# JCBrouwer/maua-style

Hardware: AMD Instinct MI355X
Metric: optimizer iterations/sec at 1024x1024 VGG-19 (higher is better)
Workload: dtype f32 (fp16x3 split-precision MFMA, fp32 accumulate)

## Files before the change

include/maua_hip.h:

```cpp
#ifndef MAUA_HIP_H
#define MAUA_HIP_H

#include <stddef.h>
#include <stdint.h>

#ifdef __cplusplus
extern "C" {
#endif

typedef void* maua_stream_t;

#define MAUA_OK 0
#define MAUA_E_INVAL (-1)
#define MAUA_E_UNSUPPORTED (-2)
#define MAUA_E_WORKSPACE (-3)

int maua_abi_version(void);
const char* maua_last_error(void);


int maua_conv_pack_filters(const float* w_oihw, float* wf, float* wb, int cout, int cin, int kh, int kw,
                           maua_stream_t stream);

size_t maua_conv_workspace_bytes(int n, int cin, int h, int w, int cout, int kh, int kw, int stride, int pad);
// ... 136 lines not shown
                                    const float* grad_scale, float* dmat, double* ledger, int slot, void* workspace, size_t workspace_bytes,
                                    maua_stream_t stream);
int maua_guided_gram_bwd_masked(const float* d_sym, const float* f, const float* guides, const float* coef, const float* mean,
                                const float* relu_mask, float* gf, int regions, int c, int64_t hw, int accumulate, maua_stream_t stream);

int maua_gram_shift_supported(int shifts, int c, int h, int w);
size_t maua_gram_shift_workspace_bytes(int shifts, int c, int h, int w);
int maua_gram_shift_fwd(const float* f, const float* mean, const int* axes, const int* deltas, const double* scales, float* gram, int shifts,
                        int c, int h, int w, void* workspace, size_t workspace_bytes, maua_stream_t stream);
int maua_gram_shift_bwd(const float* d, const float* f, const float* mean, const int* axes, const int* deltas, const double* coefs, float* gx,
                        int shifts, int c, int h, int w, int accumulate, maua_stream_t stream);

int maua_gram_flip_supported(int mirrors, int c, int h, int w);
size_t maua_gram_flip_workspace_bytes(int mirrors, int c, int h, int w);
int maua_gram_flip_fwd(const float* f, const float* mean, const int* kinds, const double* scales, float* gram, int mirrors, int c, int h, int w,
                       void* workspace, size_t workspace_bytes, maua_stream_t stream);
int maua_gram_flip_bwd(const float* d, const float* f, const float* mean, const int* kinds, const double* coefs, float* gx, int mirrors, int c,
                       int h, int w, int accumulate, maua_stream_t stream);

int maua_feat_hist_supported(int c, int h, int w, int bins, int knots);
size_t maua_feat_hist_workspace_bytes(int c, int h, int w, int bins, int knots);
size_t maua_feat_hist_state_bytes(int c, int bins);
int maua_feat_hist_fwd(const float* f, const float* table, void* state, float* loss, int c, int h, int w, int bins, int knots, void* workspace,
                       size_t workspace_bytes, maua_stream_t stream);
int maua_feat_hist_bwd(const float* f, const float* table, const void* state, const float* upstream, double coef, float* gx, int c, int h, int w,
                       int bins, int knots, int accumulate, maua_stream_t stream);

int maua_mrf_supported(int c, int h, int w, int hs, int ws, int p);
size_t maua_mrf_workspace_bytes(int c, int h, int w, int hs, int ws, int p);
size_t maua_mrf_state_bytes(int h, int w);
int maua_mrf_bank(const float* s, const int* origin, float* inv, int c, int hs, int ws, int p, maua_stream_t stream);
int maua_mrf_fwd(const float* f, const float* s, const int* origin, const float* inv, void* state, float* loss, int c, int h, int w, int hs, int ws,
                 int p, void* workspace, size_t workspace_bytes, maua_stream_t stream);
int maua_mrf_bwd(const float* f, const float* s, const int* origin, const void* state, const float* upstream, double coef, float* gx, int c, int h,
                 int w, int hs, int ws, int p, int accumulate, maua_stream_t stream);

int maua_swd_supported(int c, int d, int h, int w, int bins, int knots);
size_t maua_swd_workspace_bytes(int c, int d, int h, int w, int bins, int knots);
size_t maua_swd_state_bytes(int d, int bins);
int maua_swd_project(const float* f, const float* dirs, float* proj, void* state, int c, int d, int h, int w, int bins, void* workspace,
                     size_t workspace_bytes, maua_stream_t stream);
int maua_swd_match(float* proj_inout, const float* table, void* state, float* loss, int d, int h, int w, int bins, int knots, void* workspace,
                   size_t workspace_bytes, maua_stream_t stream);
int maua_swd_bwd(const float* g, const float* dirs_t, const float* upstream, double coef, float* gx, int c, int d, int h, int w, int accumulate,
                 maua_stream_t stream);

int maua_shift_gram_mse_ledger_supported(int shifts, int c);
int maua_shift_gram_fwd_mse_ledger(const float* f, const float* mean, const int* axes, const int* deltas, const double* scales, float* gram,
                                   int shifts, int c, int h, int w, const float* target, const double* loss_scales, const double* grad_scales,
                                   float* dmat, double* ledger, int slot, void* workspace, size_t workspace_bytes, maua_stream_t stream);
int maua_shift_gram_bwd_masked(const float* d, const float* f, const float* mean, const int* axes, const int* deltas, const double* coefs,
                               const float* relu_mask, float* gx, int shifts, int c, int h, int w, int accumulate, maua_stream_t stream);
int maua_flip_gram_mse_ledger_supported(int mirrors, int c);
int maua_flip_gram_fwd_mse_ledger(const float* f, const float* mean, const int* kinds, const double* scales, float* gram, int mirrors, int c,
                                  int h, int w, const float* target, const double* loss_scales, const double* grad_scales, float* dmat,
                                  double* ledger, int slot, void* workspace, size_t workspace_bytes, maua_stream_t stream);
int maua_flip_gram_bwd_masked(const float* d, const float* f, const float* mean, const int* kinds, const double* coefs, const float* relu_mask,
                              float* gx, int mirrors, int c, int h, int w, int accumulate, maua_stream_t stream);

int maua_tv_fwd_bwd(const float* x, float* grad, int n, int c, int h, int w, float strength, int accumulate,
                    float* loss_out, void* workspace, size_t workspace_bytes, maua_stream_t stream);

size_t maua_loss_ledger_bytes(int frames, int slots);
int maua_mse_fwd_bwd_ledger(const float* x, const float* target, float* grad, int64_t count, float loss_scale, float grad_scale,
                            int accumulate, int mask_grad_by_x, double* ledger, int slot, maua_stream_t stream);
int maua_tv_fwd_bwd_ledger(const float* x, float* grad, int n, int c, int h, int w, float strength, int accumulate,
                           double* ledger, int slot, maua_stream_t stream);
int maua_gram_mse_ledger_supported(int c);
int maua_gram_fwd_mse_ledger(const float* f, float* gram, float* row_mean_out, int c, int64_t hw, float scale, int center,
                             const float* target, float* dmat, float loss_scale, float grad_scale, double* ledger, int slot,
                             void* workspace, size_t workspace_bytes, maua_stream_t stream);
int maua_gram_partial(const float* f, float* row_mean_out, int c, int64_t hw, int center, void* workspace, size_t workspace_bytes,
                      maua_stream_t stream);
int maua_gram_partial_batch(int count, const float* const* fs, float* const* means, const int* cs, const int64_t* hws,
                            void* const* workspaces, const size_t* workspace_bytes, const int* slab_counts, maua_stream_t stream);
int maua_gram_row_means(const float* f, float* row_mean_out, int c, int64_t hw, void* workspace, size_t workspace_bytes, maua_stream_t stream);
int maua_gram_finish_mse_batch(int count, const void* const* workspaces, float* const* grams, const float* const* targets,
                               float* const* dmats, const int* cs, const int64_t* hws, const float* scales, const float* loss_scales,
                               const float* grad_scales, double* const* ledgers, const int* slots, const int* slab_counts,
                               maua_stream_t stream);
int maua_loss_ledger_sum(double* ledger, int frames, int slots, float* losses, float* totals, maua_stream_t stream);
int maua_loss_ledger_sum_f64(double* ledger, int frames, int slots, float* losses, float* totals, double* losses_f64,
                             maua_stream_t stream);

int maua_fill(float* x, int64_t count, float value, maua_stream_t stream);
size_t maua_conv_few_mfma_bank_bytes(void);
int maua_conv_pack_filters_few_mfma(const float* w_oihw, void* bank, int cout, int cin, maua_stream_t stream);
int maua_conv_few_mfma_supported(int n, int cin, int h, int w, int cout, int pad);
int maua_conv3x3_few_mfma(const float* gy, const void* bank, float* gx, int n, int cin, int h, int w, int cout, int tile, maua_stream_t stream);

int maua_space_to_depth(const float* in, float* out, int n, int c_in, int r, int h, int w, int qh, int qw, maua_stream_t stream);
int maua_depth_to_space(const float* in, float* out, int n, int c_out, int r, int qh, int qw, int h, int w, int accumulate, maua_stream_t stream);
int maua_axpy(float* y, const float* x, float alpha, int64_t count, maua_stream_t stream);
int maua_sum_small(const float* in, int count, float* out, maua_stream_t stream);

int maua_adam_step(float* x, const float* grad, float* exp_avg, float* exp_avg_sq, int64_t count, int step, float lr,
                   float beta1, float beta2, float eps, maua_stream_t stream);

size_t maua_channel_stats_workspace_bytes(int h, int w);
int maua_channel_stats(const float* x_bchw, const float* noise_bwhc, float noise_amp, int frames, int slot, int h, int w,
                       double* stats9, void* workspace, size_t workspace_bytes, maua_stream_t stream);
int maua_color_match_solve(const double* stats_target, int frames, int64_t pixels_target, const double* stats_source,
                           int64_t pixels_source, float eps, float* coef16, maua_stream_t stream);
int maua_color_match_apply(const float* x_bchw, const float* noise_bwhc, float noise_amp, const float* coef16, const float* all_coef,
                           int n_coef, float weight, int accumulate, int frames, int slot, int h, int w, float* out_bchw,
                           maua_stream_t stream);
int maua_resize_bilinear(const float* x, float* y, int planes, int h, int w, int oh, int ow, float scale_h, float scale_w,
                         maua_stream_t stream);
int maua_deprocess_u8(const float* x_bgr_chw, unsigned char* out_rgb_hwc, int h, int w, float mean_b, float mean_g, float mean_r,
                      maua_stream_t stream);

size_t maua_flow_warp_grid_workspace_bytes(int h, int w);
int maua_flow_warp_grid(const float* flow_hw2, float* grid_hw2, int h, int w, int oh, int ow, void* workspace, size_t workspace_bytes,
                        maua_stream_t stream);
int maua_grid_sample_border(const float* x, const float* grid, float* y, int n, int c, int h, int w, int oh, int ow, const float* blend,
                            double blend_a, float* init, maua_stream_t stream);
int maua_mask_u8_resize(const uint8_t* mask_hwc, float* out_chw, int h, int w, int c, int oh, int ow, maua_stream_t stream);

#define MAUA_GAUSS_WRAP_MAX_RADIUS 4096
int maua_gauss_wrap_supported(int t, int c, int h, int w, double sigma_t, double sigma_h, double sigma_w);
size_t maua_gauss_wrap_workspace_bytes(int t, int c, int h, int w, double sigma_t, double sigma_h, double sigma_w);
int maua_gauss_wrap(const float* x, float* y, int t, int c, int h, int w, double sigma_t, double sigma_h, double sigma_w, int roll_t,
                    void* workspace, size_t workspace_bytes, maua_stream_t stream);

int maua_set_tuning(const char* name, double value);
double maua_get_tuning(const char* name, double dflt);

void maua_set_split_batch_hint(int frames);
int maua_get_split_batch_hint(void);

int maua_conv_arm_workspace(void* workspace, void* counters, size_t counter_bytes, int zero, maua_stream_t stream);

size_t maua_lbfgs_state_bytes(int64_t count, int history);
int maua_lbfgs_init(void* state, size_t state_bytes, int64_t count, int history, maua_stream_t stream);
int maua_lbfgs_iterate(void* state, float* x, const float* grad, const float* loss, int64_t count, int history, float lr,
                       float tolerance_change, float tolerance_grad, maua_stream_t stream);
int maua_lbfgs_status(const void* state, int64_t count, int history, float* out5, maua_stream_t stream);

int maua_flow_levels(int h, int w, int max_levels);
int maua_flow_grey_u8(const uint8_t* rgb, float* out, int h, int w, maua_stream_t stream);
int maua_flow_pyr_down(const float* in, float* out, int h, int w, maua_stream_t stream);
int maua_flow_warp_prep(const float* i0, const float* i1, const float* u, float* fields, int h, int w, maua_stream_t stream);
int maua_flow_tvl1_step(const float* fields, const float* state_in, float* state_out, int h, int w, maua_stream_t stream);
int maua_flow_tvl1_blocked(const float* fields, const float* state_in, float* state_out, int h, int w, int k, maua_stream_t stream);
int maua_flow_median5(const float* in, float* out, int h, int w, int planes, maua_stream_t stream);
int maua_flow_upsample(const float* in, int ch, int cw, float* out, int h, int w, int planes, float scale, maua_stream_t stream);
size_t maua_flow_consistency_workspace_bytes(int h, int w);
int maua_flow_consistency(const float* flow1, const float* flow2, uint8_t* out, int h, int w, void* workspace, size_t workspace_bytes,
                          maua_stream_t stream);
size_t maua_flow_tvl1_workspace_bytes(int h, int w, int levels);
int maua_flow_tvl1(const uint8_t* rgb1, const uint8_t* rgb2, float* flow, int h, int w, int levels, int warps, int iters, int block_k,
                   void* workspace, size_t workspace_bytes, maua_stream_t stream);

int maua_nca_supported(int n, int chn, int hidden, int h, int w);
int64_t maua_nca_param_count(int chn, int hidden);
int maua_nca_step(const float* x, float* out, const float* params, int n, int chn, int hidden, int h, int w, float rate,
                  const float* rate_map, const float* mask, uint64_t seed, int64_t step, maua_stream_t stream);
size_t maua_nca_bwd_workspace_bytes(int n, int chn, int hidden, int h, int w);
int maua_nca_step_bwd(const float* x, const float* g, float* dx, const float* params, int n, int chn, int hidden, int h, int w,
                      float rate, const float* rate_map, const float* mask, uint64_t seed, int64_t step, int first, void* workspace,
                      size_t workspace_bytes, maua_stream_t stream);
int maua_nca_grad_finish(float* grad, int n, int chn, int hidden, int h, int w, const void* workspace, size_t workspace_bytes,
                         int normalize, maua_stream_t stream);

#ifdef __cplusplus
}
#endif
#endif
```

maua-style_amd/csrc/conv_api.hip:

```cpp
#include <cstdlib>
#include <cstring>

#include "conv_host.hpp"

using namespace maua;

namespace maua {
static thread_local int g_split_batch_hint = 1;
int split_batch_hint() { return g_split_batch_hint; }
static thread_local const void* g_armed_ws = nullptr;
static thread_local unsigned* g_armed_counters = nullptr;
unsigned* armed_counters(const void* workspace) { return workspace && workspace == g_armed_ws ? g_armed_counters : nullptr; }
}

namespace maua {
static const char* const g_tuning_names[] = {"conv_few_out", "few_out_ks4_below", "x3w_ks", "x3w_stagger", "x3q_ks", "x3q_min_fill", "x3q_min_chunks",
                                             "x3p_ks", "x3p_groups", "x3p_min_fill", "x3p_min_items", "x6_persist", "gram_x3", "gram_bwd_x3",
                                             "gram_t128", "gram_t128_min_hw", "p1_order", "lbfgs_vec", "lbfgs_tri", "finish_in_launch_max_ks", "x3p_order", "cot_inner", "gram_mask_reuse"};
constexpr int kTunings = sizeof(g_tuning_names) / sizeof(g_tuning_names[0]);
static double g_tuning_values[kTunings];
static bool g_tuning_set[kTunings];
static int tuning_index(const char* name) {
    for (int i = 0; i < kTunings; ++i)
        if (name && strcmp(name, g_tuning_names[i]) == 0) return i;
    return -1;
}
double tuning(const char* name, double dflt) {
    const int i = tuning_index(name);
    return i >= 0 && g_tuning_set[i] ? g_tuning_values[i] : dflt;
}
}

static inline bool mfma_geometry(int kh, int kw, int stride) {
    return stride == 1 && kh == kw && (kh == 1 || kh == 3 || kh == 5);
}
static int conv_route(const ConvArgs& a, int ks, int n, hipStream_t stream) {
    const bool few_out = tuning("conv_few_out", 1) != 0;
    if (ks == 3 && a.Cout <= 4 && a.Cin >= 16 && few_out) return conv3x3_few_out(a, n, stream);
    return conv_mfma_dispatch(a, ks, n, stream);
}

extern "C" {

int maua_set_tuning(const char* name, double value) {
    const int i = maua::tuning_index(name);
    MAUA_REQUIRE(i >= 0, MAUA_E_INVAL, "set_tuning: unknown constant %s", name ? name : "(null)");
    maua::g_tuning_values[i] = value;
    maua::g_tuning_set[i] = true;
    return MAUA_OK;
}
double maua_get_tuning(const char* name, double dflt) { return maua::tuning(name, dflt); }

int maua_conv_arm_workspace(void* workspace, void* counters, size_t counter_bytes, int zero, maua_stream_t stream) {
    if (!workspace || !counters) {
        maua::g_armed_ws = nullptr;
        maua::g_armed_counters = nullptr;
        return MAUA_OK;
    }
    MAUA_REQUIRE(counter_bytes >= (size_t)maua::ARRIVE_COUNTERS * 4 && ((size_t)counters & 15) == 0, MAUA_E_INVAL,
                 "conv_arm_workspace: needs %d bytes of 16-byte aligned counters", maua::ARRIVE_COUNTERS * 4);
    const hipError_t rc = zero ? hipMemsetAsync(counters, 0, (size_t)maua::ARRIVE_COUNTERS * 4, (hipStream_t)stream) : hipSuccess;
    if (rc != hipSuccess) {
        set_error("conv_arm_workspace: hipMemsetAsync: %s", hipGetErrorString(rc));
        return (int)rc;
    }
    maua::g_armed_ws = workspace;
    maua::g_armed_counters = (unsigned*)counters;
    return MAUA_OK;
}

void maua_set_split_batch_hint(int frames) { maua::g_split_batch_hint = frames > 0 ? frames : 1; }
int maua_get_split_batch_hint(void) { return maua::g_split_batch_hint; }

size_t maua_conv_workspace_bytes(int n, int cin, int h, int w, int cout, int kh, int kw, int stride, int pad) {
    ConvArgs a;
    if (!mfma_geometry(kh, kw, stride) || conv_geometry(a, n, cin, h, w, cout, kh, pad) != CONV_SHAPE_OK) return 0;
    if (kh == 3 && cout <= 4 && cin >= 16) return 0;
    const int ks = conv_mfma2_choose_split(a, kh, n);
    return ks > 1 ? (size_t)n * ks * cout * a.OH * a.OW * sizeof(float) : 0;
}

int maua_conv2d_fwd(const float* x, const float* in_mask, const float* wf, const float* bias, float* y, int n, int cin,
                    int h, int w, int cout, int kh, int kw, int stride, int pad, int relu, int accumulate, void* workspace,
                    size_t workspace_bytes, maua_stream_t stream) {
    MAUA_REQUIRE(x && wf && y, MAUA_E_INVAL, "conv2d_fwd: null pointer");
    MAUA_REQUIRE(conv_dims_ok(n, cin, h, w, cout, pad) && kh > 0 && kw > 0 && kh <= 64 && kw <= 64 && stride > 0 && stride <= 64, MAUA_E_INVAL,
                 "conv2d_fwd: bad dims n=%d cin=%d cout=%d h=%d w=%d k=%dx%d s=%d p=%d", n, cin, cout, h, w, kh, kw, stride,
                 pad);
    const int oh = (h + 2 * pad - kh) / stride + 1, ow = (w + 2 * pad - kw) / stride + 1;
    MAUA_REQUIRE(h + 2 * pad >= kh && w + 2 * pad >= kw, MAUA_E_UNSUPPORTED, "conv2d_fwd: input %dx%d smaller than filter", h,
                 w);
    MAUA_REQUIRE((int64_t)h * w < (1ll << 31) && (int64_t)oh * ow < (1ll << 31), MAUA_E_UNSUPPORTED,
                 "conv2d_fwd: plane too large");
    if (mfma_geometry(kh, kw, stride)) {
        ConvArgs a;
        conv_geometry(a, n, cin, h, w, cout, kh, pad);
        a.x = x;
        a.mask = in_mask;
        a.w = wf;
        a.bias = bias;
        a.y = y;
// ... 39 lines not shown
```

maua-style_amd/csrc/lbfgs.hip:

```cpp
#include <stdint.h>
#include <stdlib.h>

#include "common.hpp"

#ifndef LB_NT
#define LB_NT 1
#endif
typedef float lb_f32x4 __attribute__((ext_vector_type(4)));
#if LB_NT
__device__ __forceinline__ float lb_stream_load(const float* p) { return __builtin_nontemporal_load(p); }
__device__ __forceinline__ float4 lb_stream_load(const float4* p) {
    const lb_f32x4 v = __builtin_nontemporal_load(reinterpret_cast<const lb_f32x4*>(p));
    return make_float4(v.x, v.y, v.z, v.w);
}
#define LB_STREAM_LOAD(p) lb_stream_load(p)
#else
#define LB_STREAM_LOAD(p) (*(p))
#endif

namespace maua {

struct LbfgsHeader {
    int n_iter;
    int len;
    int head;
    int stopped;
    int cand;
    int pad0;
    float t;
    float gtd;
    double h_diag;
    float prev_loss;
    unsigned gmax_bits;
    unsigned dmax_bits;
    int pad1;
    double reserved[2];
};

constexpr int LB_EPT = 16;
constexpr int LB_WG = 256 * LB_EPT;

struct LbfgsLayout {
    int m1, nb_ids, nwg;
    size_t off_coef, off_dots, off_M, off_partial, off_gprev, off_d, off_S, off_Y, total;
};

static inline size_t align256(size_t v) { return (v + 255) & ~(size_t)255; }

static LbfgsLayout lbfgs_layout(int64_t count, int history) {
    LbfgsLayout L;
    L.m1 = history + 1;
    L.nb_ids = 2 * L.m1 + 1;
    L.nwg = (int)((count + LB_WG - 1) / LB_WG);
    size_t o = align256(sizeof(LbfgsHeader));
    L.off_coef = o;
    o = align256(o + sizeof(float) * L.nb_ids);
    L.off_dots = o;
    o = align256(o + sizeof(double) * 4 * L.nb_ids);
    L.off_M = o;
    o = align256(o + sizeof(double) * (size_t)L.nb_ids * L.nb_ids);
    L.off_partial = o;
    o = align256(o + sizeof(float) * 4 * (size_t)L.nb_ids * L.nwg);
    L.off_gprev = o;
    o = align256(o + sizeof(float) * count);
    L.off_d = o;
    o = align256(o + sizeof(float) * count);
    L.off_S = o;
    o = align256(o + sizeof(float) * count * L.m1);
    L.off_Y = o;
    o = align256(o + sizeof(float) * count * L.m1);
    L.total = o;
    return L;
}

__global__ void lbfgs_init_kernel(LbfgsHeader* h, double* M, int nb_ids, float* coef) {
    const int64_t tot = (int64_t)nb_ids * nb_ids;
    for (int64_t i = (int64_t)blockIdx.x * blockDim.x + threadIdx.x; i < tot; i += (int64_t)gridDim.x * blockDim.x) M[i] = 0.0;
    if (blockIdx.x == 0) {
        for (int i = threadIdx.x; i < nb_ids; i += blockDim.x) coef[i] = 0.f;
        if (threadIdx.x == 0) {
            h->n_iter = 0;
            h->len = 0;
            h->head = 0;
            h->stopped = 0;
            h->cand = 0;
            h->pad0 = 0;
            h->t = 0.f;
            h->gtd = 0.f;
            h->h_diag = 1.0;
            h->prev_loss = 0.f;
            h->gmax_bits = 0u;
            h->dmax_bits = 0u;
        }
    }
}

__device__ __forceinline__ void wave_reduce3_store(float a, float b, float c, float* dst, int lane) {
#pragma unroll
    for (int off = 32; off > 0; off >>= 1) {
        a += __shfl_down(a, off, 64);
        b += __shfl_down(b, off, 64);
        c += __shfl_down(c, off, 64);
    }
    if (lane == 0) {
        dst[0] = a;
        dst[1] = b;
        dst[2] = c;
    }
}

__global__ void __launch_bounds__(256)
lbfgs_pair_kernel(const LbfgsHeader* __restrict__ hdr, const float* __restrict__ g, float* __restrict__ g_prev,
                  const float* __restrict__ d, float* __restrict__ S, float* __restrict__ Y, int64_t n) {
    const bool first = hdr->n_iter == 0;
    const float t = hdr->t;
    float* sc = S + (int64_t)hdr->cand * n;
    float* yc = Y + (int64_t)hdr->cand * n;
    for (int64_t e = (int64_t)blockIdx.x * blockDim.x + threadIdx.x; e < n; e += (int64_t)gridDim.x * blockDim.x) {
        const float gv = g[e];
        sc[e] = first ? 0.f : d[e] * t;
        yc[e] = first ? 0.f : gv - g_prev[e];
        g_prev[e] = gv;
    }
}

template <bool VEC>
__global__ void __launch_bounds__(256)
lbfgs_pair_dots_kernel(LbfgsHeader* __restrict__ hdr, const float* __restrict__ g, const float* __restrict__ S,
                       const float* __restrict__ Y, float* __restrict__ partial, int64_t n, int m1) {
    extern __shared__ float lds[];
    const int nb_ids = 2 * m1 + 1;
    const int tid = threadIdx.x, lane = tid & 63, wave = tid >> 6;
    const int cand = hdr->cand, len = hdr->len, head = hdr->head;
    const int per = (len + 1 + (int)gridDim.y - 1) / (int)gridDim.y;
    const int i_begin = (int)blockIdx.y * per, i_end = min(len + 1, i_begin + per);
    if (i_begin >= i_end && blockIdx.y != 0) return;
    for (int i = tid; i < 4 * nb_ids * 4; i += 256) lds[i] = 0.f;
    __syncthreads();
    float* mine = lds + (size_t)wave * nb_ids * 4;

    const int64_t blk = (int64_t)blockIdx.x * LB_WG;
    const int rem = (int)min((int64_t)LB_WG, n - blk);
    int off[LB_EPT];
    float gv[LB_EPT], sv[LB_EPT], yv[LB_EPT];
    {
        const float* gB = g + blk;
        const float* sB = S + (int64_t)cand * n + blk;
        const float* yB = Y + (int64_t)cand * n + blk;
#pragma unroll
        for (int k = 0; k < LB_EPT; ++k) {
            const int e = VEC ? 4 * (tid + 256 * (k >> 2)) + (k & 3) : tid + 256 * k;
            const bool ok = e < rem;
            off[k] = ok ? e : 0;
            gv[k] = ok ? gB[off[k]] : 0.f;
            sv[k] = ok ? sB[off[k]] : 0.f;
            yv[k] = ok ? yB[off[k]] : 0.f;
        }
    }
#pragma unroll 1
    for (int i = i_begin; i < i_end; ++i) {
        const int p = i < len ? (head + i) % m1 : cand;
        const float* sp = S + (int64_t)p * n + blk;
        const float* yp = Y + (int64_t)p * n + blk;
        float ls[LB_EPT], ly[LB_EPT];
        if constexpr (VEC) {
#pragma unroll
            for (int k = 0; k < LB_EPT; k += 4) {
                const float4 a = LB_STREAM_LOAD(reinterpret_cast<const float4*>(sp + off[k]));
                const float4 b = LB_STREAM_LOAD(reinterpret_cast<const float4*>(yp + off[k]));
                ls[k] = a.x, ls[k + 1] = a.y, ls[k + 2] = a.z, ls[k + 3] = a.w;
                ly[k] = b.x, ly[k + 1] = b.y, ly[k + 2] = b.z, ly[k + 3] = b.w;
            }
        } else {
#pragma unroll
            for (int k = 0; k < LB_EPT; ++k) {
                ls[k] = LB_STREAM_LOAD(sp + off[k]);
                ly[k] = LB_STREAM_LOAD(yp + off[k]);
            }
        }
        float a0 = 0.f, a1 = 0.f, a2 = 0.f, b0 = 0.f, b1 = 0.f, b2 = 0.f;
#pragma unroll
        for (int k = 0; k < LB_EPT; ++k) {
            a0 = fmaf(ls[k], sv[k], a0);
            a1 = fmaf(ls[k], yv[k], a1);
            a2 = fmaf(ls[k], gv[k], a2);
            b0 = fmaf(ly[k], sv[k], b0);
            b1 = fmaf(ly[k], yv[k], b1);
            b2 = fmaf(ly[k], gv[k], b2);
        }
        wave_reduce3_store(a0, a1, a2, mine + 4 * p, lane);
        wave_reduce3_store(b0, b1, b2, mine + 4 * (m1 + p), lane);
    }
    if (blockIdx.y == 0) {
        float sg = 0.f, yg = 0.f, gg = 0.f, g1 = 0.f, gm = 0.f;
#pragma unroll
        for (int k = 0; k < LB_EPT; ++k) {
            sg = fmaf(sv[k], gv[k], sg);
            yg = fmaf(yv[k], gv[k], yg);
            gg = fmaf(gv[k], gv[k], gg);
            g1 += fabsf(gv[k]);
            gm = fmaxf(gm, fabsf(gv[k]));
        }
        wave_reduce3_store(sg, yg, gg, mine + 4 * (2 * m1), lane);
        g1 = wave_sum(g1);
        gm = wave_max_nonneg(gm);
        if (lane == 0) {
// ... 447 lines not shown
#pragma unroll EPT >= 16 ? 2 : 8
    for (int i = 0; i < len; ++i) {
        const int p = (head + i) % m1;
        const float cs = coef[p], cy = coef[m1 + p];
        const float* sp = S + (int64_t)p * n + blk;
        const float* yp = Y + (int64_t)p * n + blk;
#pragma unroll
        for (int k = 0; k < EPT; ++k) {
            const int e = tid + 256 * k;
            const int ec = e < rem ? e : 0;
            acc[k] = fmaf(cy, LB_STREAM_LOAD(yp + ec), fmaf(cs, LB_STREAM_LOAD(sp + ec), acc[k]));
        }
    }
    float* dB = d + blk;
    float* xB = x + blk;
    float dm = 0.f;
#pragma unroll
    for (int k = 0; k < EPT; ++k) {
        const int e = tid + 256 * k;
        if (e < rem) {
            dB[e] = acc[k];
            dm = fmaxf(dm, fabsf(acc[k] * t));
            if (!stopped) xB[e] = fmaf(t, acc[k], xB[e]);
        }
    }
    dm = wave_max_nonneg(dm);
    if ((tid & 63) == 0 && !stopped) atomicMax(dmax_bits, __float_as_uint(dm));
}

__global__ void __launch_bounds__(256)
lbfgs_combine_v4_kernel(const LbfgsHeader* __restrict__ hdr, const float* __restrict__ coef, const float* __restrict__ g,
                        const float* __restrict__ S, const float* __restrict__ Y, float* __restrict__ d, float* __restrict__ x,
                        int64_t n, int m1, unsigned* __restrict__ dmax_bits) {
    const int len = hdr->len, head = hdr->head, stopped = hdr->stopped;
    const float t = hdr->t;
    const int64_t e = ((int64_t)blockIdx.x * blockDim.x + threadIdx.x) * 4;
    const bool ok = e < n;
    const int64_t ec = ok ? e : 0;
    const float cg = coef[2 * m1];
    const float4 gv = *reinterpret_cast<const float4*>(g + ec);
    float4 acc = make_float4(cg * gv.x, cg * gv.y, cg * gv.z, cg * gv.w);
#pragma unroll 8
    for (int i = 0; i < len; ++i) {
        const int p = (head + i) % m1;
        const float cs = coef[p], cy = coef[m1 + p];
        const float4 sv = LB_STREAM_LOAD(reinterpret_cast<const float4*>(S + (int64_t)p * n + ec));
        const float4 yv = LB_STREAM_LOAD(reinterpret_cast<const float4*>(Y + (int64_t)p * n + ec));
        acc.x = fmaf(cy, yv.x, fmaf(cs, sv.x, acc.x));
        acc.y = fmaf(cy, yv.y, fmaf(cs, sv.y, acc.y));
        acc.z = fmaf(cy, yv.z, fmaf(cs, sv.z, acc.z));
        acc.w = fmaf(cy, yv.w, fmaf(cs, sv.w, acc.w));
    }
    float dm = 0.f;
    if (ok) {
        *reinterpret_cast<float4*>(d + e) = acc;
        dm = fmaxf(fmaxf(fabsf(acc.x * t), fabsf(acc.y * t)), fmaxf(fabsf(acc.z * t), fabsf(acc.w * t)));
        if (!stopped) {
            float4 xv = *reinterpret_cast<const float4*>(x + e);
            xv.x = fmaf(t, acc.x, xv.x);
            xv.y = fmaf(t, acc.y, xv.y);
            xv.z = fmaf(t, acc.z, xv.z);
            xv.w = fmaf(t, acc.w, xv.w);
            *reinterpret_cast<float4*>(x + e) = xv;
        }
    }
    dm = wave_max_nonneg(dm);
    if ((threadIdx.x & 63) == 0 && !stopped) atomicMax(dmax_bits, __float_as_uint(dm));
}

__global__ void lbfgs_status_kernel(const LbfgsHeader* __restrict__ hdr, float* __restrict__ out) {
    if (threadIdx.x == 0) {
        out[0] = (float)hdr->n_iter;
        out[1] = (float)hdr->len;
        out[2] = (float)hdr->stopped;
        out[3] = hdr->gtd;
        out[4] = hdr->t;
    }
}

}

using namespace maua;

extern "C" {

size_t maua_lbfgs_state_bytes(int64_t count, int history) {
    if (count <= 0 || history <= 0 || history > 254 || count >= (1ll << 36)) return 0;
    return lbfgs_layout(count, history).total;
}

int maua_lbfgs_init(void* state, size_t state_bytes, int64_t count, int history, maua_stream_t stream) {
    MAUA_REQUIRE(state && count > 0 && count < (1ll << 36) && history > 0 && history <= 254, MAUA_E_INVAL, "lbfgs_init: bad args");
    MAUA_REQUIRE(2 * (history + 1) + 1 <= 512, MAUA_E_UNSUPPORTED, "lbfgs_init: history %d too large (at most 254)", history);
    const LbfgsLayout L = lbfgs_layout(count, history);
    MAUA_REQUIRE(state_bytes >= L.total, MAUA_E_WORKSPACE, "lbfgs_init: state %zu < %zu bytes", state_bytes, L.total);
    char* b = (char*)state;
    hipLaunchKernelGGL(lbfgs_init_kernel, dim3(64), dim3(256), 0, (hipStream_t)stream, (LbfgsHeader*)b,
                       (double*)(b + L.off_M), L.nb_ids, (float*)(b + L.off_coef));
    return check_launch("lbfgs_init_kernel");
}

int maua_lbfgs_iterate(void* state, float* x, const float* grad, const float* loss, int64_t count, int history, float lr,
                       float tolerance_change, float tolerance_grad, maua_stream_t stream) {
    MAUA_REQUIRE(state && x && grad && count > 0 && count < (1ll << 36) && history > 0 && history <= 254, MAUA_E_INVAL, "lbfgs_iterate: bad args");
    const LbfgsLayout L = lbfgs_layout(count, history);
    char* b = (char*)state;
    LbfgsHeader* hdr = (LbfgsHeader*)b;
    float* coef = (float*)(b + L.off_coef);
    double* dots = (double*)(b + L.off_dots);
    double* M = (double*)(b + L.off_M);
    float* partial = (float*)(b + L.off_partial);
    float* g_prev = (float*)(b + L.off_gprev);
    float* d = (float*)(b + L.off_d);
    float* S = (float*)(b + L.off_S);
    float* Y = (float*)(b + L.off_Y);
    hipStream_t s = (hipStream_t)stream;
    const size_t lds1 = sizeof(float) * 4 * L.nb_ids * 4;
    MAUA_REQUIRE(lds1 <= 64 * 1024 && L.nb_ids <= 512, MAUA_E_UNSUPPORTED, "lbfgs_iterate: history %d too large (at most 254)", history);
    int pg = (int)((count + 1023) / 1024);
    if (pg > 2048) pg = 2048;
    hipLaunchKernelGGL(lbfgs_pair_kernel, dim3(pg), dim3(256), 0, s, hdr, grad, g_prev, d, S, Y, count);
    int rc = check_launch("lbfgs_pair_kernel");
    if (rc) return rc;
    int groups = (1024 + L.nwg - 1) / L.nwg;
    if (groups > L.m1) groups = L.m1;
    const bool aligned = count % 4 == 0 && (((uintptr_t)x | (uintptr_t)grad) & 15) == 0;
    const bool vec_on = tuning("lbfgs_vec", 1) != 0;
    if (aligned && vec_on)
        hipLaunchKernelGGL(lbfgs_pair_dots_kernel<true>, dim3(L.nwg, groups), dim3(256), lds1, s, hdr, grad, S, Y, partial, count, L.m1);
    else
        hipLaunchKernelGGL(lbfgs_pair_dots_kernel<false>, dim3(L.nwg, groups), dim3(256), lds1, s, hdr, grad, S, Y, partial, count, L.m1);
    rc = check_launch("lbfgs_pair_dots_kernel");
    if (rc) return rc;
    hipLaunchKernelGGL(lbfgs_finish_dots_kernel, dim3(L.nb_ids), dim3(256), 0, s, hdr, partial, dots, L.nwg, L.nb_ids, L.m1);
    rc = check_launch("lbfgs_finish_dots_kernel");
    if (rc) return rc;
    const size_t lds3 = sizeof(double) * 2 * (L.m1 + 1);
    const size_t lds_tri = sizeof(double) * ((size_t)L.m1 * (L.m1 | 1) + 2 * (size_t)L.m1 + 384 + 16);
    const bool tri_on = tuning("lbfgs_tri", 1) != 0;
    if (tri_on && L.m1 <= 128 && lds_tri <= 144 * 1024) {
        static unsigned long long attr_set = 0;
        (void)opt_in_dynamic_lds(reinterpret_cast<const void*>(lbfgs_coeffs_tri_kernel), 144 * 1024, &attr_set);
        hipLaunchKernelGGL(lbfgs_coeffs_tri_kernel, dim3(1), dim3(256), lds_tri, s, hdr, dots, M, coef, L.m1, history, lr,
                           tolerance_change, tolerance_grad, loss);
    } else if (L.nb_ids <= 256)
        hipLaunchKernelGGL(lbfgs_coeffs_kernel<4>, dim3(1), dim3(64), lds3, s, hdr, dots, M, coef, L.m1, history, lr,
                           tolerance_change, tolerance_grad, loss);
    else
        hipLaunchKernelGGL(lbfgs_coeffs_kernel<8>, dim3(1), dim3(64), lds3, s, hdr, dots, M, coef, L.m1, history, lr,
                           tolerance_change, tolerance_grad, loss);
    rc = check_launch("lbfgs_coeffs_kernel");
    if (rc) return rc;
    auto combine = [&](auto kernel, int ept) {
        hipLaunchKernelGGL(kernel, dim3((unsigned)((count + 256 * ept - 1) / (256 * ept))), dim3(256), 0, s, hdr, coef, grad, S, Y, d,
                           x, count, L.m1, &hdr->dmax_bits);
    };
    if (count >= 256 * 16 * 512) combine(lbfgs_combine_kernel<16>, 16);
    else if (aligned && vec_on)
        hipLaunchKernelGGL(lbfgs_combine_v4_kernel, dim3((unsigned)((count / 4 + 63) / 64)), dim3(64), 0, s, hdr, coef, grad, S, Y, d,
                           x, count, L.m1, &hdr->dmax_bits);
    else if (count >= 256 * 4 * 512) combine(lbfgs_combine_kernel<4>, 4);
    else combine(lbfgs_combine_kernel<1>, 1);
    return check_launch("lbfgs_combine_kernel");
}

#ifdef LB_STAMP
int maua_lbfgs_read_stamps(unsigned long long* host16) {
    return (int)hipMemcpyFromSymbol(host16, HIP_SYMBOL(g_lb_stamps), sizeof(unsigned long long) * 16);
}
#endif

int maua_lbfgs_status(const void* state, int64_t count, int history, float* out5, maua_stream_t stream) {
    MAUA_REQUIRE(state && out5 && count > 0 && history > 0 && history <= 254, MAUA_E_INVAL, "lbfgs_status: bad args");
    hipLaunchKernelGGL(lbfgs_status_kernel, dim3(1), dim3(64), 0, (hipStream_t)stream, (const LbfgsHeader*)state, out5);
    return check_launch("lbfgs_status_kernel");
}

}
```

maua-style_amd/csrc/pointwise.hip:

```cpp
#include <stdarg.h>

#include "common.hpp"

namespace maua {

static thread_local char g_err[512] = "";

void set_error(const char* fmt, ...) {
    va_list ap;
    va_start(ap, fmt);
    vsnprintf(g_err, sizeof(g_err), fmt, ap);
    va_end(ap);
}

__global__ void finish_sum_kernel(const double* __restrict__ partial, int n, float scale, float* __restrict__ out) {
    __shared__ double scratch[16];
    double v = 0.0;
    for (int i = threadIdx.x; i < n; i += blockDim.x) v += partial[i];
    v = block_sum(v, scratch);
    if (threadIdx.x == 0) out[0] = (float)(v * (double)scale);
}

constexpr int LEDGER_GROUPS = 4;
__global__ void __launch_bounds__(256 * LEDGER_GROUPS)
loss_ledger_sum_kernel(double* __restrict__ ledger, int slots, float* __restrict__ losses, float* __restrict__ total,
                       double* __restrict__ exact) {
    __shared__ double scratch[LEDGER_GROUPS][4];
    __shared__ float kept[1 << 12];
    double* led = ledger + (int64_t)blockIdx.x * slots * LEDGER_STRIDE;
    float* out = losses + (int64_t)blockIdx.x * slots;
    const int grp = threadIdx.x >> 8, t = threadIdx.x & 255, lane = t & 63, wave = t >> 6;
    constexpr int PER = LEDGER_MAX / 256;
    for (int s0 = 0; s0 < slots; s0 += LEDGER_GROUPS) {
        const int s = s0 + grp;
        const bool have = s < slots;
        const double* rec = led + (int64_t)(have ? s : 0) * LEDGER_STRIDE;
        double part[PER];
#pragma unroll
        for (int i = 0; i < PER; ++i) part[i] = rec[2 + t + 256 * i];
        const int n = have ? min((int)rec[0], LEDGER_MAX) : 0;
        double v = 0.0;
#pragma unroll
        for (int i = 0; i < PER; ++i) v += t + 256 * i < n ? part[i] : 0.0;
        v = wave_sum(v);
        if (lane == 0) scratch[grp][wave] = v;
        __syncthreads();
        if (t == 0 && have) {
            if (n > 0) {
                double r = 0.0;
                for (int i = 0; i < 4; ++i) r += scratch[grp][i];
                const double scl = rec[1];
                kept[s] = (float)(r * scl);
                out[s] = kept[s];
                if (exact) exact[(int64_t)blockIdx.x * slots + s] = r * scl;
                led[(int64_t)s * LEDGER_STRIDE] = 0.0;
            } else {
                kept[s] = out[s];
            }
        }
        __syncthreads();
    }
    if (threadIdx.x == 0) {
        float tot = 0.f;
        for (int s = 0; s < slots; ++s) tot += kept[s];
        total[blockIdx.x] = tot;
    }
}

__global__ void pack_filters_kernel(const float* __restrict__ w, float* __restrict__ wf, float* __restrict__ wb, int cout,
                                    int cin, int kh, int kw) {
    const int64_t total = (int64_t)cout * cin * kh * kw;
    for (int64_t e = (int64_t)blockIdx.x * blockDim.x + threadIdx.x; e < total; e += (int64_t)gridDim.x * blockDim.x) {
        int64_t r = e;
        const int kx = (int)(r % kw);
        r /= kw;
        const int ky = (int)(r % kh);
        r /= kh;
        const int ci = (int)(r % cin);
        const int co = (int)(r / cin);
        const float v = w[e];
        if (wf) wf[((int64_t)(ky * kw + kx) * cin + ci) * cout + co] = v;
        if (wb) wb[((int64_t)((kh - 1 - ky) * kw + (kw - 1 - kx)) * cout + co) * cin + ci] = v;
    }
}

__global__ void relu_fwd_kernel(float* __restrict__ x, int64_t n) {
    for (int64_t i = (int64_t)blockIdx.x * blockDim.x + threadIdx.x; i < n; i += (int64_t)gridDim.x * blockDim.x)
        x[i] = x[i] > 0.f ? x[i] : 0.f;
}

__global__ void relu_bwd_kernel(const float* __restrict__ gy, const float* __restrict__ y, float* __restrict__ gx,
                                int64_t n) {
    for (int64_t i = (int64_t)blockIdx.x * blockDim.x + threadIdx.x; i < n; i += (int64_t)gridDim.x * blockDim.x)
        gx[i] = y[i] > 0.f ? gy[i] : 0.f;
}

__global__ void fill_kernel(float* __restrict__ x, int64_t n, float v) {
    for (int64_t i = (int64_t)blockIdx.x * blockDim.x + threadIdx.x; i < n; i += (int64_t)gridDim.x * blockDim.x) x[i] = v;
}

__global__ void axpy_kernel(float* __restrict__ y, const float* __restrict__ x, float a, int64_t n) {
    for (int64_t i = (int64_t)blockIdx.x * blockDim.x + threadIdx.x; i < n; i += (int64_t)gridDim.x * blockDim.x)
        y[i] = fmaf(a, x[i], y[i]);
}

__global__ void sum_small_kernel(const float* __restrict__ in, int n, float* __restrict__ out) {
    if (threadIdx.x == 0 && blockIdx.x == 0) {
        float s = 0.f;
        for (int i = 0; i < n; ++i) s += in[i];
        out[0] = s;
    }
}

__device__ __forceinline__ int window_argmax(const float* __restrict__ plane, int H, int W, int oy, int ox, int k, int s) {
    const int y0 = oy * s, x0 = ox * s;
    const int y1 = min(y0 + k, H), x1 = min(x0 + k, W);
    int best = y0 * W + x0;
    float bv = plane[best];
    for (int yy = y0; yy < y1; ++yy)
        for (int xx = x0; xx < x1; ++xx) {
            const float v = plane[yy * W + xx];
            if (v > bv || v != v) {
                bv = v;
                best = yy * W + xx;
            }
        }
    return best;
}

__global__ void pool_fwd_kernel(const float* __restrict__ x, float* __restrict__ y, int64_t planes, int H, int W, int OH,
                                int OW, int k, int s, int mode) {
    const int64_t total = planes * OH * OW;
    for (int64_t e = (int64_t)blockIdx.x * blockDim.x + threadIdx.x; e < total; e += (int64_t)gridDim.x * blockDim.x) {
        const int ox = (int)(e % OW);
        const int oy = (int)((e / OW) % OH);
        const int64_t pl = e / ((int64_t)OW * OH);
        const float* plane = x + pl * H * W;
        if (mode == 0) {
            y[e] = plane[window_argmax(plane, H, W, oy, ox, k, s)];
        } else {
            const int y0 = oy * s, x0 = ox * s, y1 = min(y0 + k, H), x1 = min(x0 + k, W);
            float acc = 0.f;
            for (int yy = y0; yy < y1; ++yy)
                for (int xx = x0; xx < x1; ++xx) acc += plane[yy * W + xx];
            y[e] = acc / (float)((y1 - y0) * (x1 - x0));
        }
    }
}

// ... 416 lines not shown
        hipLaunchKernelGGL(pool2x2_bwd_codes_kernel<false>, dim3((w / 2 + 255) / 256, h / 2, n * c), dim3(256), 0, (hipStream_t)stream, gy,
                           codes, gx, h, w, w / 2, relu_mask);
    return check_launch("pool2x2_bwd_codes_kernel");
}

size_t maua_reduce_workspace_bytes(int64_t count) { return (size_t)reduce_blocks(count, 1024) * sizeof(double); }

int maua_mse_fwd_bwd(const float* x, const float* target, float* grad, int64_t count, float loss_scale, float grad_scale,
                     int accumulate, int mask_grad_by_x, float* loss_out, void* workspace, size_t workspace_bytes,
                     maua_stream_t stream) {
    MAUA_REQUIRE(x && target && loss_out && workspace && count > 0, MAUA_E_INVAL, "mse_fwd_bwd: bad args");
    const int nb = reduce_blocks(count, 1024);
    MAUA_REQUIRE(workspace_bytes >= nb * sizeof(double), MAUA_E_WORKSPACE, "mse_fwd_bwd: workspace %zu < %zu",
                 workspace_bytes, nb * sizeof(double));
    hipLaunchKernelGGL(mse_kernel, dim3(nb), dim3(256), 0, (hipStream_t)stream, x, target, grad, count, grad_scale,
                       accumulate, mask_grad_by_x, (double*)workspace, (double*)nullptr, 0.f);
    int rc = check_launch("mse_kernel");
    if (rc) return rc;
    hipLaunchKernelGGL(finish_sum_kernel, dim3(1), dim3(256), 0, (hipStream_t)stream, (const double*)workspace, nb,
                       loss_scale, loss_out);
    return check_launch("finish_sum_kernel");
}

int maua_mse_weighted_fwd_bwd(const float* x, const float* weights, const float* target, float* grad, int64_t planes,
                              int64_t plane, int weight_planes, float loss_scale, float grad_scale, int accumulate,
                              float* loss_out, void* workspace, size_t workspace_bytes, maua_stream_t stream) {
    MAUA_REQUIRE(x && weights && target && loss_out && workspace && planes > 0 && plane > 0, MAUA_E_INVAL,
                 "mse_weighted_fwd_bwd: bad args");
    MAUA_REQUIRE(weight_planes == 1 || weight_planes == planes, MAUA_E_INVAL,
                 "mse_weighted_fwd_bwd: weights need 1 or %lld planes, got %d", (long long)planes, weight_planes);
    const int64_t count = planes * plane;
    const int nb = reduce_blocks(count, 1024);
    MAUA_REQUIRE(workspace_bytes >= nb * sizeof(double), MAUA_E_WORKSPACE, "mse_weighted_fwd_bwd: workspace too small");
    hipLaunchKernelGGL(mse_weighted_kernel, dim3(nb), dim3(256), 0, (hipStream_t)stream, x, weights, target, grad, count, plane,
                       weight_planes, grad_scale, accumulate, (double*)workspace);
    int rc = check_launch("mse_weighted_kernel");
    if (rc) return rc;
    hipLaunchKernelGGL(finish_sum_kernel, dim3(1), dim3(256), 0, (hipStream_t)stream, (const double*)workspace, nb,
                       loss_scale, loss_out);
    return check_launch("finish_sum_kernel");
}

int maua_tv_fwd_bwd(const float* x, float* grad, int n, int c, int h, int w, float strength, int accumulate,
                    float* loss_out, void* workspace, size_t workspace_bytes, maua_stream_t stream) {
    MAUA_REQUIRE(x && loss_out && workspace && conv_dims_ok(n, c, h, w, 1, 0), MAUA_E_INVAL, "tv_fwd_bwd: bad args");
    const int64_t count = (int64_t)n * c * h * w;
    const int nb = reduce_blocks(count, 1024);
    MAUA_REQUIRE(workspace_bytes >= nb * sizeof(double), MAUA_E_WORKSPACE, "tv_fwd_bwd: workspace too small");
    hipLaunchKernelGGL(tv_kernel, dim3(nb), dim3(256), 0, (hipStream_t)stream, x, grad, (int64_t)n * c, h, w, strength,
                       accumulate, (double*)workspace, (double*)nullptr);
    int rc = check_launch("tv_kernel");
    if (rc) return rc;
    hipLaunchKernelGGL(finish_sum_kernel, dim3(1), dim3(256), 0, (hipStream_t)stream, (const double*)workspace, nb, strength,
                       loss_out);
    return check_launch("finish_sum_kernel");
}

size_t maua_loss_ledger_bytes(int frames, int slots) {
    if (frames <= 0 || slots <= 0 || frames > (1 << 16) || slots > (1 << 12)) return 0;
    return (size_t)frames * slots * LEDGER_STRIDE * sizeof(double);
}

int maua_mse_fwd_bwd_ledger(const float* x, const float* target, float* grad, int64_t count, float loss_scale, float grad_scale,
                            int accumulate, int mask_grad_by_x, double* ledger, int slot, maua_stream_t stream) {
    MAUA_REQUIRE(x && target && ledger && slot >= 0 && slot < (1 << 28) && count > 0, MAUA_E_INVAL, "mse_fwd_bwd_ledger: bad args");
    const int nb = reduce_blocks(count, 1024);
    double* rec = ledger + (int64_t)slot * LEDGER_STRIDE;
    hipLaunchKernelGGL(mse_kernel, dim3(nb), dim3(256), 0, (hipStream_t)stream, x, target, grad, count, grad_scale, accumulate,
                       mask_grad_by_x, rec + 2, rec, loss_scale);
    return check_launch("mse_kernel");
}

int maua_tv_fwd_bwd_ledger(const float* x, float* grad, int n, int c, int h, int w, float strength, int accumulate,
                           double* ledger, int slot, maua_stream_t stream) {
    MAUA_REQUIRE(x && ledger && slot >= 0 && slot < (1 << 28) && conv_dims_ok(n, c, h, w, 1, 0), MAUA_E_INVAL, "tv_fwd_bwd_ledger: bad args");
    const int64_t count = (int64_t)n * c * h * w;
    const int nb = reduce_blocks(count, 1024);
    double* rec = ledger + (int64_t)slot * LEDGER_STRIDE;
    hipLaunchKernelGGL(tv_kernel, dim3(nb), dim3(256), 0, (hipStream_t)stream, x, grad, (int64_t)n * c, h, w, strength, accumulate,
                       rec + 2, rec);
    return check_launch("tv_kernel");
}

int maua_loss_ledger_sum(double* ledger, int frames, int slots, float* losses, float* totals, maua_stream_t stream) {
    MAUA_REQUIRE(ledger && losses && totals && frames > 0 && frames <= (1 << 16) && slots > 0 && slots <= (1 << 12), MAUA_E_INVAL,
                 "loss_ledger_sum: bad args");
    hipLaunchKernelGGL(loss_ledger_sum_kernel, dim3(frames), dim3(256 * LEDGER_GROUPS), 0, (hipStream_t)stream, ledger, slots, losses, totals,
                       (double*)nullptr);
    return check_launch("loss_ledger_sum_kernel");
}

int maua_loss_ledger_sum_f64(double* ledger, int frames, int slots, float* losses, float* totals, double* losses_f64,
                             maua_stream_t stream) {
    MAUA_REQUIRE(ledger && losses && totals && losses_f64 && frames > 0 && frames <= (1 << 16) && slots > 0 && slots <= (1 << 12),
                 MAUA_E_INVAL, "loss_ledger_sum_f64: bad args");
    hipLaunchKernelGGL(loss_ledger_sum_kernel, dim3(frames), dim3(256 * LEDGER_GROUPS), 0, (hipStream_t)stream, ledger, slots, losses, totals,
                       losses_f64);
    return check_launch("loss_ledger_sum_kernel");
}

int maua_depth_to_space(const float* in, float* out, int n, int c_out, int r, int qh, int qw, int h, int w, int accumulate, maua_stream_t stream) {
    MAUA_REQUIRE(in && out && n > 0 && c_out > 0 && r > 0 && r <= 16 && qh > 0 && qw > 0 && h > 0 && w > 0 && (int64_t)n * c_out <= 65535 && h <= 65535,
                 MAUA_E_INVAL, "depth_to_space: bad args");
    hipLaunchKernelGGL(depth_to_space_kernel, dim3((w + 255) / 256, h, n * c_out), dim3(256), 0, (hipStream_t)stream, in, out, c_out, r, qh, qw, h, w, accumulate);
    return check_launch("depth_to_space_kernel");
}

int maua_space_to_depth(const float* in, float* out, int n, int c_in, int r, int h, int w, int qh, int qw, maua_stream_t stream) {
    MAUA_REQUIRE(in && out && n > 0 && c_in > 0 && r > 0 && r <= 16 && qh > 0 && qw > 0 && h > 0 && w > 0 && (int64_t)n * c_in * r * r <= 65535 && qh <= 65535,
                 MAUA_E_INVAL, "space_to_depth: bad args");
    hipLaunchKernelGGL(space_to_depth_kernel, dim3((qw + 255) / 256, qh, n * c_in * r * r), dim3(256), 0, (hipStream_t)stream, in, out, c_in, r, qh, qw, h, w);
    return check_launch("space_to_depth_kernel");
}

int maua_fill(float* x, int64_t count, float value, maua_stream_t stream) {
    MAUA_REQUIRE(x && count > 0, MAUA_E_INVAL, "fill: bad args");
    hipLaunchKernelGGL(fill_kernel, dim3(ew_grid(count)), dim3(256), 0, (hipStream_t)stream, x, count, value);
    return check_launch("fill_kernel");
}

int maua_axpy(float* y, const float* x, float alpha, int64_t count, maua_stream_t stream) {
    MAUA_REQUIRE(x && y && count > 0, MAUA_E_INVAL, "axpy: bad args");
    hipLaunchKernelGGL(axpy_kernel, dim3(ew_grid(count)), dim3(256), 0, (hipStream_t)stream, y, x, alpha, count);
    return check_launch("axpy_kernel");
}

int maua_sum_small(const float* in, int count, float* out, maua_stream_t stream) {
    MAUA_REQUIRE(in && out && count > 0, MAUA_E_INVAL, "sum_small: bad args");
    hipLaunchKernelGGL(sum_small_kernel, dim3(1), dim3(64), 0, (hipStream_t)stream, in, count, out);
    return check_launch("sum_small_kernel");
}

int maua_adam_step(float* x, const float* grad, float* exp_avg, float* exp_avg_sq, int64_t count, int step, float lr,
                   float beta1, float beta2, float eps, maua_stream_t stream) {
    MAUA_REQUIRE(x && grad && exp_avg && exp_avg_sq && count > 0 && step >= 1, MAUA_E_INVAL, "adam_step: bad args");
    const double bc1 = 1.0 - pow((double)beta1, step), bc2 = 1.0 - pow((double)beta2, step);
    const float step_size = (float)((double)lr / bc1);
    const float sqrt_bc2 = (float)sqrt(bc2);
    hipLaunchKernelGGL(adam_kernel, dim3(ew_grid(count)), dim3(256), 0, (hipStream_t)stream, x, grad, exp_avg, exp_avg_sq,
                       count, (float)(1.0 - (double)beta1), beta2, (float)(1.0 - (double)beta2), sqrt_bc2, step_size,
                       eps);
    return check_launch("adam_kernel");
}

}
```

maua-style_amd/engine.py:

```python
import contextlib
import os

import torch

import hip
import loss as loss_mod
import models as models_mod
import plan


class UnsupportedNet(RuntimeError):
    """The module sequence contains something the fused plan does not cover (callers fall back to running the
    modules one by one, which still executes on the GPU through the same kernels)."""


def _scale_grad_coeff(incoming, strength):
    g = float(incoming)
    return g / (abs(g) + 1e-8) * strength * strength


def guided_coefficients(strength, video_style_factor, normalize, channels, active, has_target):
    s, vsf = strength, video_style_factor
    dyn = vsf > 0
    lw = s + (vsf * s if dyn else 0.0)
# ... 481 lines not shown
            if gd is None:
                raise UnsupportedNet("guided StyleLoss runs on the module path")
            if gd["target"] is None:
                if m.guided_target is None:
                    raise RuntimeError(f"{getattr(m, 'name', 'StyleLoss')}: guided style target not captured")
                raise ValueError("guided StyleLoss: content and style guides must name the same regions")
            return True
        if m.shift_factor > 0 and not getattr(m, "terms_engine", False):
            raise UnsupportedNet("shifted StyleLoss runs on the module path")
        if m.target.nelement() == 0:
            raise RuntimeError(f"{m.name}: style target not captured")
        if shapes_src[0] == 1 and m.video_style_factor > 0 and m.video_target.nelement() != 0 \
                and m.video_target.shape != m.target.shape:
            raise UnsupportedNet("dynamic style target of another shape")
        return True

    def _arm(self):
        if self.ws_counters is None:
            hip.conv_arm_workspace(None)
            return
        if self.ws_armed_epoch != (self.ws.data_ptr(), self.ws_counters.data_ptr()):
            hip.conv_arm_workspace(self.ws, self.ws_counters)
            self.ws_armed_epoch = (self.ws.data_ptr(), self.ws_counters.data_ptr())
        else:
            hip.conv_arm_workspace(self.ws, self.ws_counters, zero=False)

    def fork(self):
        if self.side:
            self.ev_main.record()
            for st in self.side:
                st.wait_event(self.ev_main)

    def join(self):
        cur = torch.cuda.current_stream()
        for st, ev in zip(self.side, self.ev_side):
            ev.record(st)
            cur.wait_event(ev)

    def _gram_ws(self, s, c, hw, dev):
        need = hip.gram_workspace_bytes(c, hw)
        t = self._gram_wsp.get(id(s))
        if t is None or t.numel() < need or t.device != dev:
            t = torch.empty(need, dtype=torch.uint8, device=dev)
            self._gram_wsp[id(s)] = t
        return t

    def frame_stream(self, b):
        if not self.side:
            import contextlib
            return contextlib.nullcontext(), self.ws
        k = b % len(self.side)
        return torch.cuda.stream(self.side[k]), self.side_ws[k]

    def _timed(self, tag, flops, nbytes, fn):
        if self.timer is None:
            return fn()
        e0, e1 = torch.cuda.Event(enable_timing=True), torch.cuda.Event(enable_timing=True)
        e0.record()
        out = fn()
        e1.record()
        self.timer.append((tag, flops, nbytes, e0, e1))
        return out

    @staticmethod
    def _conv_work(s, in_shape, out_shape, backward):
        _, cin, h, w = in_shape
        _, cout, oh, ow = out_shape
        flops = 2 * cin * cout * s.k * s.k * oh * ow
        wbytes = (cin * cout * s.k * s.k + cout) * 4
        ib, ob = cin * h * w * 4, cout * oh * ow * 4
        nbytes = (ob + ob + wbytes + ib) if backward else (ib + wbytes + ob)
        return flops, nbytes

    def _image_gram_now(self, s, shape):
        st, _ = self.image_gram[id(s)]
        return self.gram_batch_on and self.gram_partial_batch_on and self._active(st, self.act[s.dst].shape)

    def image_gram_slabs(self, style_step):
        return next(n for st, n in self.image_gram.values() if st is style_step)

    def _x6_ok(self, s, produced_channels):
        return self.use_x6 and s.k == 3 and s.stride == 1 and s.pad <= 2 and produced_channels >= plan.get_int("split_min_produced")

    def _run(self, x):
        hip.set_split_batch_hint(self.batch_hint)
        self._arm()
        a, g = self.act, self.gbuf
        a[0] = x
        hip.fill_(self.slots_all, 0.0)
        forked = False
        batch = []
        emitted = set()
        for s in self.steps:
            if s.kind == "conv":
                fl, nb = self._conv_work(s, a[s.src].shape, a[s.dst].shape, False)
                if id(s) in self.fused_pool:
                    ps = self.fused_pool[id(s)]
                    self._timed("conv3x3_split_fwd", fl, nb, lambda: models_mod.conv3x3_relu_pool(
                        a[s.src], s.mod, a[ps.dst], self.pool_codes[id(ps)], workspace=self.ws))
                elif id(s) in self.image_gram and self._image_gram_now(s, a[s.src].shape):
                    st, _ = self.image_gram[id(s)]
                    gws = self._gram_ws(st, 64, a[s.dst].shape[2] * a[s.dst].shape[3], x.device)
                    models_mod._route("conv_image", a[s.src], s.mod.out_channels, s.pad, False, "27 (channel, tap) pairs as K, bf16x6", relu=True, gram_slabs=True)
                    self._timed("conv3x3_split_fwd", fl, nb, lambda: hip.conv3x3_image_gram(a[s.src], s.mod.bank_image(), s.pad, a[s.dst], gws))
                    emitted.add(id(st))
                elif self.x6_fwd and self._x6_ok(s, s.mod.out_channels):
                    self._timed("conv3x3_split_fwd", fl, nb, lambda: models_mod.conv3x3_mfma(
                        a[s.src], s.mod, False, out=a[s.dst], relu=s.relu, workspace=self.ws))
                elif self.x6_fwd and models_mod.conv1x1_is_mfma(s.mod, False):
                    self._timed("conv_1x1_fwd", fl, nb, lambda: models_mod.conv1x1_mfma(
                        a[s.src], s.mod, False, out=a[s.dst], relu=s.relu, workspace=self.ws))
                elif self.x6_fwd and models_mod.conv5x5_is_mfma(s.mod, False):
                    self._timed("conv_5x5_fwd", fl, nb, lambda: models_mod.conv5x5_mfma(
                        a[s.src], s.mod, False, out=a[s.dst], relu=s.relu, workspace=self.ws))
                elif id(s) in self.strided_fwd_sites:
                    self._timed("conv_other_fwd", fl, nb, lambda: models_mod.conv_strided_fwd_as_3x3(
                        a[s.src], s.mod, a[s.dst], s.relu, self.strided_fwd_sites[id(s)], workspace=self.ws))
                else:
                    wf, _ = s.mod.banks()
                    models_mod._route("conv2d_fwd", a[s.src], s.mod.out_channels, s.pad, False, "direct / fp32 MFMA", relu=s.relu)
                    self._timed("conv_other_fwd", fl, nb, lambda: hip.conv2d_fwd(
                        a[s.src], wf, s.mod.bias_device(), s.k, s.stride, s.pad, s.relu, out=a[s.dst], workspace=self.ws))
            elif s.kind == "relu":
                hip.relu_(a[s.src])
            elif s.kind == "pool":
                if id(s) in self.pooled_by_conv:
                    pass
                elif id(s) in self.pool_codes:
                    hip.pool2x2_fwd_codes(a[s.src], a[s.dst], self.pool_codes[id(s)])
                else:
                    hip.pool2d_fwd(a[s.src], s.k, s.stride, s.ceil, s.mode, out=a[s.dst])
            elif s.kind == "style" and id(s) in self.guided:
                if self._active(s, a[s.src].shape):
                    f, gd = a[s.src], self.guided[id(s)]
                    lg, cov = gd["lg"], bool(s.mod.use_covariance)
                    c, n, r = f.shape[1], f[0].nelement(), gd["lg"].g.shape[0]
                    self._timed("gram_fwd", 2 * c * c * (n // c), n * 4 + r * c * c * 4, lambda: hip.gram_guided_fwd_mse_ledger(
                        f, lg.g, lg.scale, cov, lg.mass, self.gram[id(s)], self.mean[id(s)], gd["target"], self.dmat[id(s)], gd["loss_scale"],
                        gd["grad_scale"], self.ledger[0], s.slot, workspace=self.ws))
            elif s.kind == "style" and id(s) in self.term_steps:
                if self._active(s, a[s.src].shape):
                    f, td = a[s.src], self.term_steps[id(s)]
                    c, n = f.shape[1], f[0].nelement()
                    lw, gw = self._coefficients(s)
                    ls, gs, ssc, lf, gf, fsc = td["coef"]
                    self._timed("gram_fwd", 2 * c * c * (n // c), n * 4 + c * c * 4, lambda: hip.gram_fwd_mse_ledger(
                        f, 1.0 / n, s.mod.use_covariance, self.gram[id(s)], self.mean[id(s)], s.mod.target, self.dmat[id(s)],
                        lw / (c * c), gw * 4.0 / (c * c) / n, self.ledger[0], s.slot, workspace=self.ws))
                    if td["shifts"]:
                        k = len(td["shifts"])
                        self._timed("gram_fwd", 2 * k * c * c * (n // c), n * 4 + 3 * k * c * c * 4, lambda: hip.gram_shift_fwd_mse_ledger(
                            f, td["shifts"], ssc, None, td["s_gram"][:k], td["s_target"][:k], td["s_dmat"][:k], ls, gs, self.ledger[0],
                            td["shift_slot"], workspace=self.ws))
                    if lf:
                        k = len(lf)
                        self._timed("gram_fwd", 2 * k * c * c * (n // c), n * 4 + 3 * k * c * c * 4, lambda: hip.gram_flip_fwd_mse_ledger(
                            f, td["kinds"], fsc, self.mean[id(s)], td["f_gram"], td["f_target"], td["f_dmat"], lf, gf, self.ledger[0],
                            td["flip_slot"], workspace=self.ws))
            elif s.kind == "style" and self.independent and a[s.src].shape[0] > 1 and self._active(s, a[s.src].shape):
                f = a[s.src]
                c, n = f.shape[1], f[0].nelement()
                lw, gw = self._coefficients(s)
                fs = self.fused_style.get(id(s))
                self.fork()
                for b in range(f.shape[0]):
                    mean_b = self.mean[id(s)][b] if s.mod.use_covariance else None
                    ctx, wsb = self.frame_stream(b)
                    with ctx:
                        if self.ledger is not None and hip.gram_mse_ledger_supported(c):
                            self._timed("gram_fwd", 2 * c * c * (n // c), n * 4 + c * c * 4, lambda: hip.gram_fwd_mse_ledger(
                                f[b:b + 1], 1.0 / n, s.mod.use_covariance, self.gram[id(s)][b], mean_b, s.mod.target,
                                self.dmat[id(s)][b], lw / (c * c), gw * 4.0 / (c * c) / n, self.ledger[b], s.slot, workspace=wsb))
# ... 218 lines not shown
                                        lambda: fn(acc or i > 0, rm if i == len(todo) - 1 else None))
                    else:
                        self._timed("gram_bwd", 2 * c * c * (n // c), n * 4 * 3 + c * c * 4, lambda: hip.gram_bwd(
                            self.dmat[id(s)], f, self.mean[id(s)], g[s.src], acc, workspace=self.ws, relu_mask=rm))
                    cur = s.src
            elif s.kind == "content":
                if self._active(s, a[s.src].shape):
                    lw, gw = self._coefficients(s)
                    n = a[s.src].nelement()
                    if s.mod.weights is not None:
                        hip.mse_weighted_fwd_bwd(a[s.src], s.mod.weights, s.mod.target, g[s.src], lw / n, gw * 2.0 / n,
                                                 cur == s.src, self.slots[s.slot:s.slot + 1], workspace=self.ws)
                    elif self.ledger is not None:
                        hip.mse_fwd_bwd_ledger(a[s.src], s.mod.target, g[s.src], lw / n, gw * 2.0 / n, cur == s.src, self.ledger[0],
                                               s.slot, mask_grad_by_x=premask(s))
                    else:
                        hip.mse_fwd_bwd(a[s.src], s.mod.target, g[s.src], lw / n, gw * 2.0 / n, cur == s.src,
                                        self.slots[s.slot:s.slot + 1], workspace=self.ws, mask_grad_by_x=premask(s))
                    cur = s.src
            elif s.kind == "tv":
                if self.ledger is not None:
                    hip.tv_fwd_bwd_ledger(a[0], g[0], s.mod.strength, cur == 0, self.ledger[0], s.slot)
                else:
                    hip.tv_fwd_bwd(a[0], g[0], s.mod.strength, cur == 0, self.slots[s.slot:s.slot + 1], workspace=self.ws)
                cur = 0
            elif cur is None:
                continue
            elif s.kind == "conv":
                assert cur == s.dst
                fl, nb = self._conv_work(s, a[s.src].shape, a[s.dst].shape, True)
                im = a[s.src] if premask(s) else None
                fg = self.fused_gram.get(id(s))
                with_gram = fg is not None and self._active(fg[0], a[s.src].shape) and premask(fg[0])
                up = self.fused_unpool.get(id(s))
                if up is not None:
                    c, n = a[s.src].shape[1], a[s.src][0].nelement()
                    self._timed("conv3x3_split_bwd", fl + (2 * c * c * (n // c) if with_gram else 0), nb, lambda: models_mod.conv3x3_bwd_from_pooled(
                        g[up.dst], self.pool_codes[id(up)], premask(up), s.mod, g[s.src], out_relu_mask=a[s.src] if with_gram else im,
                        dmat_bank=fg[1] if with_gram else None, dmat_inv_scale=fg[2] if with_gram else None, workspace=self.ws))
                    if with_gram:
                        fused_done.add(id(fg[0]))
                elif with_gram:
                    c, n = a[s.src].shape[1], a[s.src][0].nelement()
                    self._timed("conv3x3_split_bwd", fl + 2 * c * c * (n // c), nb, lambda: models_mod.conv3x3_bwd_with_gram(
                        g[s.dst], s.mod, a[s.src], fg[1], fg[2], out=g[s.src], workspace=self.ws))
                    fused_done.add(id(fg[0]))
                elif self.x6_bwd and self._x6_ok(s, s.mod.in_channels):
                    self._timed("conv3x3_split_bwd", fl, nb, lambda: models_mod.conv3x3_mfma(
                        g[s.dst], s.mod, True, out=g[s.src], out_relu_mask=im, workspace=self.ws, pool_group=id(s) in self.pool_groups))
                elif self.x6_bwd and models_mod.conv1x1_is_mfma(s.mod, True):
                    self._timed("conv_1x1_bwd", fl, nb, lambda: models_mod.conv1x1_mfma(
                        g[s.dst], s.mod, True, out=g[s.src], out_relu_mask=im, workspace=self.ws))
                elif self.x6_bwd and models_mod.conv5x5_is_mfma(s.mod, True):
                    self._timed("conv_5x5_bwd", fl, nb, lambda: models_mod.conv5x5_mfma(
                        g[s.dst], s.mod, True, out=g[s.src], out_relu_mask=im, workspace=self.ws))
                elif im is None and models_mod.conv_few_is_mfma(s.mod, *g[s.dst].shape[0:1], *g[s.dst].shape[2:]):
                    self._timed("conv_other_bwd", fl, nb, lambda: models_mod.conv_few_mfma(g[s.dst], s.mod, g[s.src]))
                elif id(s) in self.strided_sites and im is None:
                    self._timed("conv_other_bwd", fl, nb, lambda: models_mod.conv_strided_bwd_as_3x3(
                        g[s.dst], s.mod, g[s.src], workspace=self.ws, sites=self.strided_sites[id(s)]))
                else:
                    _, wb = s.mod.banks()
                    models_mod._route("conv3x3_few_out" if s.k == 3 and s.stride == 1 and s.mod.in_channels <= 4 and s.mod.out_channels >= 16 else "conv2d_bwd_data",
                                      g[s.dst], s.mod.in_channels, s.k - 1 - s.pad, True, "direct / fp32 MFMA", mask=im is not None)
                    self._timed("conv_other_bwd", fl, nb, lambda: hip.conv2d_bwd_data(
                        g[s.dst], None, wb, s.mod.weight.detach(), a[s.src].shape, s.k, s.stride, s.pad, out=g[s.src],
                        in_relu_mask=im, workspace=self.ws))
                cur = s.src
            elif s.kind == "relu":
                hip.relu_bwd(g[s.src], a[s.src], out=g[s.src])
            elif s.kind == "pool":
                assert cur == s.dst
                if id(s) in self.unpooled_by_conv:
                    pass
                elif id(s) in self.pool_codes:
                    hip.pool2x2_bwd_codes(g[s.dst], self.pool_codes[id(s)], g[s.src], premask(s))
                else:
                    hip.pool2d_bwd(g[s.dst], a[s.src], s.k, s.stride, s.ceil, s.mode, out=g[s.src],
                                   relu_mask_by_x=premask(s))
                cur = s.src
        if cur != 0:
            hip.fill_(g[0], 0.0)
        if self.ledger is not None:
            hip.loss_ledger_sum(self.ledger, self.slots_all, self.total, self.slots_f64)
            for s in self.steps:
                td = self.term_steps.get(id(s))
                if td is not None and self._active(s, a[s.src].shape):
                    for e in (td["shift_slot"], td["flip_slot"]):
                        if e is not None:
                            self.slots_all[s.slot:s.slot + 1].add_(self.slots_all[e:e + 1])
                            if self.slots_f64 is not None:
                                self.slots_f64.view(-1)[s.slot:s.slot + 1].add_(self.slots_f64.view(-1)[e:e + 1])
            return
        if indep:
            for b in range(x.shape[0]):
                hip.sum_small(self.slots_all[b], self.total[b:b + 1])
            return
        hip.sum_small(self.slots_all, self.total)
        for s in self.steps:
            if id(s) in self.terms:
                t = self.terms[id(s)]
                self.slots_all[s.slot:s.slot + 1] = self.slots_all[t[0]:t[-1] + 1].sum(0, keepdim=True)

    def capture_content(self, x):
        self._prepare(x)
        a = self.act
        a[0] = x
        want = [s for s in self.steps if s.kind == "content" and "temporal" not in getattr(s.mod, "name", "")]
        last = max((self.steps.index(s) for s in want), default=-1)
        for s in self.steps[:last + 1]:
            if s.kind == "conv":
                if id(s) in self.fused_pool:
                    ps = self.fused_pool[id(s)]
                    models_mod.conv3x3_relu_pool(a[s.src], s.mod, a[ps.dst], self.pool_codes[id(ps)], workspace=self.ws)
                elif self.x6_fwd and self._x6_ok(s, s.mod.out_channels):
                    models_mod.conv3x3_mfma(a[s.src], s.mod, False, out=a[s.dst], relu=s.relu, workspace=self.ws)
                elif self.x6_fwd and models_mod.conv1x1_is_mfma(s.mod, False):
                    models_mod.conv1x1_mfma(a[s.src], s.mod, False, out=a[s.dst], relu=s.relu, workspace=self.ws)
                elif self.x6_fwd and models_mod.conv5x5_is_mfma(s.mod, False):
                    models_mod.conv5x5_mfma(a[s.src], s.mod, False, out=a[s.dst], relu=s.relu, workspace=self.ws)
                elif id(s) in self.strided_fwd_sites:
                    models_mod.conv_strided_fwd_as_3x3(a[s.src], s.mod, a[s.dst], s.relu, self.strided_fwd_sites[id(s)], workspace=self.ws)
                else:
                    wf, _ = s.mod.banks()
                    hip.conv2d_fwd(a[s.src], wf, s.mod.bias_device(), s.k, s.stride, s.pad, s.relu, out=a[s.dst],
                                   workspace=self.ws)
            elif s.kind == "relu":
                hip.relu_(a[s.src])
            elif s.kind == "pool":
                if id(s) not in self.pooled_by_conv:
                    hip.pool2d_fwd(a[s.src], s.k, s.stride, s.ceil, s.mode, out=a[s.dst])
        for s in want:
            t = getattr(s.mod, "target", None)
            if torch.is_tensor(t) and t.shape == a[s.src].shape and t.device == a[s.src].device and t.dtype == a[s.src].dtype:
                t.copy_(a[s.src])
            else:
                s.mod.target = a[s.src].detach().clone()

    def _graph_key(self):
        def sig(t):
            return None if t is None or not torch.is_tensor(t) else (t.data_ptr(), tuple(t.shape))
        key = []
        for s in self.steps:
            m = s.mod
            if s.kind in ("tv", "content", "style"):
                key.append((s.kind, id(m), getattr(m, "mode", None), float(m.strength), bool(getattr(m, "normalize", False)),
                            sig(getattr(m, "target", None)), sig(getattr(m, "video_target", None)), sig(getattr(m, "weights", None)),
                            float(getattr(m, "video_style_factor", 0.0)), bool(getattr(m, "use_covariance", False))))
                gd = getattr(self, "guided", {}).get(id(s))
                if gd is not None:
                    lg = gd["lg"]
                    key.append(("guided", sig(getattr(m, "guide", None)), sig(lg.g), sig(lg.scale), sig(lg.mass), sig(gd["target"]), gd["coef"]))
                td = getattr(self, "term_steps", {}).get(id(s))
                key.append(("terms_engine", bool(getattr(m, "terms_engine", False))))
                if td is not None:
                    key.append(("terms", td["sig"] and tuple(p[:2] for p in td["sig"]), tuple(td["shifts"]), td["kinds"], float(m.shift_factor),
                                float(m.flip_factor), float(m.rotation_factor), td["coef"], td["err"]))
            elif s.kind == "conv":
                key.append((id(m), m.weight.data_ptr(), m.weight._version))
        key.append(("hint", self.batch_hint, self.independent))
        return tuple(key)

    def feval(self, x, capture=False):
        self._prepare(x)
        if not capture:
            self._run(x)
            return self.slots, self.total, self.gbuf[0]
# ... 43 lines not shown
```

maua-style_amd/hip.py:

```python
import ctypes
import threading
import os
import sys

import torch

HERE = os.path.dirname(os.path.abspath(__file__))
LIB_PATH = os.path.join(HERE, "libmaua_hip.so")

c_f = ctypes.c_float
c_i = ctypes.c_int
c_i64 = ctypes.c_int64
c_p = ctypes.c_void_p
c_sz = ctypes.c_size_t
c_u64 = ctypes.c_uint64

SIGNATURES = {
    "maua_abi_version": (c_i, []),
    "maua_last_error": (ctypes.c_char_p, []),
    "maua_conv_pack_filters": (c_i, [c_p, c_p, c_p, c_i, c_i, c_i, c_i, c_p]),
    "maua_conv_workspace_bytes": (c_sz, [c_i, c_i, c_i, c_i, c_i, c_i, c_i, c_i, c_i]),
    "maua_conv2d_fwd": (c_i, [c_p, c_p, c_p, c_p, c_p, c_i, c_i, c_i, c_i, c_i, c_i, c_i, c_i, c_i, c_i, c_i, c_p, c_sz, c_p]),
    "maua_conv2d_bwd_data": (c_i, [c_p, c_p, c_p, c_p, c_p, c_p, c_i, c_i, c_i, c_i, c_i, c_i, c_i, c_i, c_i, c_i, c_p, c_sz,
                                   c_p]),
# ... 58 lines not shown
    "maua_mrf_supported": (c_i, [c_i, c_i, c_i, c_i, c_i, c_i]),
    "maua_mrf_workspace_bytes": (c_sz, [c_i, c_i, c_i, c_i, c_i, c_i]),
    "maua_mrf_state_bytes": (c_sz, [c_i, c_i]),
    "maua_mrf_bank": (c_i, [c_p, c_p, c_p, c_i, c_i, c_i, c_i, c_p]),
    "maua_mrf_fwd": (c_i, [c_p, c_p, c_p, c_p, c_p, c_p, c_i, c_i, c_i, c_i, c_i, c_i, c_p, c_sz, c_p]),
    "maua_mrf_bwd": (c_i, [c_p, c_p, c_p, c_p, c_p, ctypes.c_double, c_p, c_i, c_i, c_i, c_i, c_i, c_i, c_i, c_p]),
    "maua_swd_supported": (c_i, [c_i, c_i, c_i, c_i, c_i, c_i]),
    "maua_swd_workspace_bytes": (c_sz, [c_i, c_i, c_i, c_i, c_i, c_i]),
    "maua_swd_state_bytes": (c_sz, [c_i, c_i]),
    "maua_swd_project": (c_i, [c_p, c_p, c_p, c_p, c_i, c_i, c_i, c_i, c_i, c_p, c_sz, c_p]),
    "maua_swd_match": (c_i, [c_p, c_p, c_p, c_p, c_i, c_i, c_i, c_i, c_i, c_p, c_sz, c_p]),
    "maua_swd_bwd": (c_i, [c_p, c_p, c_p, ctypes.c_double, c_p, c_i, c_i, c_i, c_i, c_i, c_p]),
    "maua_guided_gram_mse_ledger_supported": (c_i, [c_i, c_i]),
    "maua_guided_gram_fwd_mse_ledger": (c_i, [c_p, c_p, c_p, c_p, c_p, c_p, c_i, c_i, c_i64, c_i, c_p, c_p, c_p, c_p, c_p, c_i, c_p, c_sz, c_p]),
    "maua_guided_gram_bwd_masked": (c_i, [c_p, c_p, c_p, c_p, c_p, c_p, c_p, c_i, c_i, c_i64, c_i, c_p]),
    "maua_shift_gram_mse_ledger_supported": (c_i, [c_i, c_i]),
    "maua_shift_gram_fwd_mse_ledger": (c_i, [c_p, c_p, c_p, c_p, c_p, c_p, c_i, c_i, c_i, c_i, c_p, c_p, c_p, c_p, c_p, c_i, c_p, c_sz, c_p]),
    "maua_shift_gram_bwd_masked": (c_i, [c_p, c_p, c_p, c_p, c_p, c_p, c_p, c_p, c_i, c_i, c_i, c_i, c_i, c_p]),
    "maua_flip_gram_mse_ledger_supported": (c_i, [c_i, c_i]),
    "maua_flip_gram_fwd_mse_ledger": (c_i, [c_p, c_p, c_p, c_p, c_p, c_i, c_i, c_i, c_i, c_p, c_p, c_p, c_p, c_p, c_i, c_p, c_sz, c_p]),
    "maua_flip_gram_bwd_masked": (c_i, [c_p, c_p, c_p, c_p, c_p, c_p, c_p, c_i, c_i, c_i, c_i, c_i, c_p]),
    "maua_tv_fwd_bwd": (c_i, [c_p, c_p, c_i, c_i, c_i, c_i, c_f, c_i, c_p, c_p, c_sz, c_p]),
    "maua_fill": (c_i, [c_p, c_i64, c_f, c_p]),
    "maua_depth_to_space": (c_i, [c_p, c_p, c_i, c_i, c_i, c_i, c_i, c_i, c_i, c_i, c_p]),
    "maua_conv_few_mfma_bank_bytes": (c_sz, []),
    "maua_conv_pack_filters_few_mfma": (c_i, [c_p, c_p, c_i, c_i, c_p]),
    "maua_conv_few_mfma_supported": (c_i, [c_i, c_i, c_i, c_i, c_i, c_i]),
    "maua_conv3x3_few_mfma": (c_i, [c_p, c_p, c_p, c_i, c_i, c_i, c_i, c_i, c_i, c_p]),
    "maua_space_to_depth": (c_i, [c_p, c_p, c_i, c_i, c_i, c_i, c_i, c_i, c_i, c_p]),
    "maua_axpy": (c_i, [c_p, c_p, c_f, c_i64, c_p]),
    "maua_sum_small": (c_i, [c_p, c_i, c_p, c_p]),
    "maua_adam_step": (c_i, [c_p, c_p, c_p, c_p, c_i64, c_i, c_f, c_f, c_f, c_f, c_p]),
    "maua_channel_stats_workspace_bytes": (c_sz, [c_i, c_i]),
    "maua_channel_stats": (c_i, [c_p, c_p, c_f, c_i, c_i, c_i, c_i, c_p, c_p, c_sz, c_p]),
    "maua_color_match_solve": (c_i, [c_p, c_i, c_i64, c_p, c_i64, c_f, c_p, c_p]),
    "maua_color_match_apply": (c_i, [c_p, c_p, c_f, c_p, c_p, c_i, c_f, c_i, c_i, c_i, c_i, c_i, c_p, c_p]),
    "maua_resize_bilinear": (c_i, [c_p, c_p, c_i, c_i, c_i, c_i, c_i, c_f, c_f, c_p]),
    "maua_deprocess_u8": (c_i, [c_p, c_p, c_i, c_i, c_f, c_f, c_f, c_p]),
    "maua_flow_warp_grid_workspace_bytes": (c_sz, [c_i, c_i]),
    "maua_flow_warp_grid": (c_i, [c_p, c_p, c_i, c_i, c_i, c_i, c_p, c_sz, c_p]),
    "maua_grid_sample_border": (c_i, [c_p, c_p, c_p, c_i, c_i, c_i, c_i, c_i, c_i, c_p, ctypes.c_double, c_p, c_p]),
    "maua_mask_u8_resize": (c_i, [c_p, c_p, c_i, c_i, c_i, c_i, c_i, c_p]),
    "maua_gauss_wrap_supported": (c_i, [c_i, c_i, c_i, c_i, ctypes.c_double, ctypes.c_double, ctypes.c_double]),
    "maua_gauss_wrap_workspace_bytes": (c_sz, [c_i, c_i, c_i, c_i, ctypes.c_double, ctypes.c_double, ctypes.c_double]),
    "maua_gauss_wrap": (c_i, [c_p, c_p, c_i, c_i, c_i, c_i, ctypes.c_double, ctypes.c_double, ctypes.c_double, c_i, c_p, c_sz, c_p]),
    "maua_set_tuning": (c_i, [ctypes.c_char_p, ctypes.c_double]),
    "maua_get_tuning": (ctypes.c_double, [ctypes.c_char_p, ctypes.c_double]),
    "maua_set_split_batch_hint": (None, [c_i]),
    "maua_conv_arm_workspace": (c_i, [c_p, c_p, c_sz, c_i, c_p]),
    "maua_get_split_batch_hint": (c_i, []),
    "maua_conv_x3w_split": (c_i, [c_i, c_i, c_i, c_i, c_i, c_i]),
    "maua_conv_x3q_bank_bytes": (c_sz, [c_i, c_i]),
    "maua_conv_pack_filters_x3q": (c_i, [c_p, c_p, c_p, c_i, c_i, c_f, c_p]),
    "maua_conv_x3q_supported": (c_i, [c_i, c_i, c_i, c_i]),
    "maua_conv_x3q_workspace_bytes": (c_sz, [c_i, c_i, c_i, c_i, c_i, c_i]),
    "maua_conv_x3q_split": (c_i, [c_i, c_i, c_i, c_i, c_i, c_i]),
    "maua_conv_x3q_preferred": (c_i, [c_i, c_i, c_i, c_i, c_i, c_i]),
    "maua_conv3x3_x3q": (c_i, [c_p, c_p, c_f, c_p, c_p, c_p, c_i, c_i, c_i, c_i, c_i, c_i, c_i, c_i, c_p, c_sz, c_p]),
    "maua_conv3x3_x3q_relu_pool": (c_i, [c_p, c_p, c_f, c_p, c_p, c_p, c_i, c_i, c_i, c_i, c_i, c_i, c_p, c_sz, c_p]),
    "maua_conv3x3_x3q_unpool": (c_i, [c_p, c_p, c_i, c_p, c_f, c_p, c_p, c_i, c_i, c_i, c_i, c_i, c_i, c_p, c_sz, c_p]),
    "maua_conv_x3p_supported": (c_i, [c_i, c_i, c_i, c_i, c_i]),
    "maua_conv_x3p_split": (c_i, [c_i, c_i, c_i, c_i, c_i, c_i]),
    "maua_conv_x3p_workspace_bytes": (c_sz, [c_i, c_i, c_i, c_i, c_i, c_i]),
    "maua_conv_x3p_preferred": (c_i, [c_i, c_i, c_i, c_i, c_i, c_i]),
    "maua_conv_x3p_set_max_groups": (c_i, [c_i]),
    "maua_conv3x3_x3p": (c_i, [c_p, c_p, c_i, c_p, c_f, c_p, c_p, c_p, c_p, c_p, c_p, c_i, c_i, c_i, c_i, c_i, c_i, c_i, c_p, c_sz, c_p]),
    "maua_conv3x3_x3w_relu_pool": (c_i, [c_p, c_p, c_f, c_p, c_p, c_p, c_i, c_i, c_i, c_i, c_i, c_i, c_p, c_sz, c_p]),
    "maua_conv_x3w_dmat_bank_bytes": (c_sz, [c_i]),
    "maua_conv_pack_dmat_x3w": (c_i, [c_p, c_i, c_p, c_p, c_p]),
    "maua_conv_pack_dmat_x3w_batch": (c_i, [c_i, c_p, c_p, c_p, c_p, c_p]),
    "maua_conv3x3_x3w_gram": (c_i, [c_p, c_p, c_f, c_p, c_p, c_p, c_p, c_i, c_i, c_i, c_i, c_i, c_i, c_i, c_p, c_sz, c_p]),
    "maua_conv3x3_x3w_unpool": (c_i, [c_p, c_p, c_i, c_p, c_f, c_p, c_p, c_p, c_p, c_i, c_i, c_i, c_i, c_i, c_i, c_p, c_sz, c_p]),
    "maua_loss_ledger_bytes": (c_sz, [c_i, c_i]),
    "maua_mse_fwd_bwd_ledger": (c_i, [c_p, c_p, c_p, c_i64, c_f, c_f, c_i, c_i, c_p, c_i, c_p]),
    "maua_tv_fwd_bwd_ledger": (c_i, [c_p, c_p, c_i, c_i, c_i, c_i, c_f, c_i, c_p, c_i, c_p]),
    "maua_gram_mse_ledger_supported": (c_i, [c_i]),
    "maua_gram_fwd_mse_ledger": (c_i, [c_p, c_p, c_p, c_i, c_i64, c_f, c_i, c_p, c_p, c_f, c_f, c_p, c_i, c_p, c_sz, c_p]),
    "maua_gram_partial": (c_i, [c_p, c_p, c_i, c_i64, c_i, c_p, c_sz, c_p]),
    "maua_gram_finish_mse_batch": (c_i, [c_i, c_p, c_p, c_p, c_p, c_p, c_p, c_p, c_p, c_p, c_p, c_p, c_p, c_p]),
    "maua_gram_partial_batch": (c_i, [c_i, c_p, c_p, c_p, c_p, c_p, c_p, c_p, c_p]),
    "maua_gram_row_means": (c_i, [c_p, c_p, c_i, c_i64, c_p, c_sz, c_p]),
    "maua_loss_ledger_sum": (c_i, [c_p, c_i, c_i, c_p, c_p, c_p]),
    "maua_loss_ledger_sum_f64": (c_i, [c_p, c_i, c_i, c_p, c_p, c_p, c_p]),
    "maua_lbfgs_state_bytes": (c_sz, [c_i64, c_i]),
    "maua_lbfgs_init": (c_i, [c_p, c_sz, c_i64, c_i, c_p]),
    "maua_lbfgs_iterate": (c_i, [c_p, c_p, c_p, c_p, c_i64, c_i, c_f, c_f, c_f, c_p]),
    "maua_lbfgs_status": (c_i, [c_p, c_i64, c_i, c_p, c_p]),
    "maua_flow_levels": (c_i, [c_i, c_i, c_i]),
    "maua_flow_grey_u8": (c_i, [c_p, c_p, c_i, c_i, c_p]),
    "maua_flow_pyr_down": (c_i, [c_p, c_p, c_i, c_i, c_p]),
    "maua_flow_warp_prep": (c_i, [c_p, c_p, c_p, c_p, c_i, c_i, c_p]),
    "maua_flow_tvl1_step": (c_i, [c_p, c_p, c_p, c_i, c_i, c_p]),
    "maua_flow_tvl1_blocked": (c_i, [c_p, c_p, c_p, c_i, c_i, c_i, c_p]),
    "maua_flow_median5": (c_i, [c_p, c_p, c_i, c_i, c_i, c_p]),
    "maua_flow_upsample": (c_i, [c_p, c_i, c_i, c_p, c_i, c_i, c_i, c_f, c_p]),
    "maua_flow_consistency_workspace_bytes": (c_sz, [c_i, c_i]),
    "maua_flow_consistency": (c_i, [c_p, c_p, c_p, c_i, c_i, c_p, c_sz, c_p]),
    "maua_flow_tvl1_workspace_bytes": (c_sz, [c_i, c_i, c_i]),
    "maua_flow_tvl1": (c_i, [c_p, c_p, c_p, c_i, c_i, c_i, c_i, c_i, c_i, c_p, c_sz, c_p]),
    "maua_nca_supported": (c_i, [c_i, c_i, c_i, c_i, c_i]),
    "maua_nca_param_count": (c_i64, [c_i, c_i]),
    "maua_nca_step": (c_i, [c_p, c_p, c_p, c_i, c_i, c_i, c_i, c_i, c_f, c_p, c_p, c_u64, c_i64, c_p]),
    "maua_nca_bwd_workspace_bytes": (c_sz, [c_i, c_i, c_i, c_i, c_i]),
    "maua_nca_step_bwd": (c_i, [c_p, c_p, c_p, c_p, c_i, c_i, c_i, c_i, c_i, c_f, c_p, c_p, c_u64, c_i64, c_i, c_p, c_sz, c_p]),
    "maua_nca_grad_finish": (c_i, [c_p, c_i, c_i, c_i, c_i, c_i, c_p, c_sz, c_i, c_p]),
}


class HipError(RuntimeError):
    pass


_lib = None


def lib():
    global _lib, LIB_PATH
    if _lib is None:
        LIB_PATH = os.environ.get("MAUA_HIP_LIB", LIB_PATH)
        if not os.path.exists(LIB_PATH):
            raise HipError(
                f"{LIB_PATH} not found: build it with `python maua-style_amd/build_native.py` "
                "(this package has no CPU or PyTorch fallback)")
        try:
            L = ctypes.CDLL(LIB_PATH)
        except OSError as e:
            raise HipError(f"cannot load {LIB_PATH}: {e}") from e
        for name, (res, args) in SIGNATURES.items():
            fn = getattr(L, name)
            fn.restype = res
            fn.argtypes = args
        _lib = L
        here = os.path.dirname(os.path.abspath(__file__))
        if here not in sys.path:
            sys.path.insert(0, here)
        import plan
        plan.forward_to_library(L)
        plan.warn_ignored()
    return _lib


def apply_plan():
    here = os.path.dirname(os.path.abspath(__file__))
    if here not in sys.path:
        sys.path.insert(0, here)
    import plan
    plan.forward_to_library(lib())


def _check(rc, what):
    if rc != 0:
        msg = lib().maua_last_error().decode(errors="replace")
        raise HipError(f"{what} failed (rc={rc}): {msg}")


def _ptr(t):
    if t is None:
        return None
    if not t.is_cuda:
        raise HipError("libmaua_hip needs ROCm device tensors (got a CPU tensor): there is no CPU path")
    if t.dtype != torch.float32 and t.dtype != torch.uint8 and t.dtype != torch.float64:
        raise HipError(f"unsupported dtype {t.dtype}")
    if not t.is_contiguous():
        raise HipError("tensor must be contiguous")
    return t.data_ptr()


def _stream():
    try:
# ... 464 lines not shown
    need = gram_workspace_bytes(c, hw)
    workspace = _ws(workspace, need, f.device)
    _check(lib().maua_gram_fwd(_ptr(_f32(f, "f")), _ptr(out), _ptr(mean_out) if center else None, c, hw, float(scale),
                               int(center), workspace.data_ptr(), workspace.numel() * workspace.element_size(),
                               _stream()), "maua_gram_fwd")
    return out, (mean_out if center else None)


def loss_ledger(frames, slots, device):
    n = lib().maua_loss_ledger_bytes(int(frames), int(slots)) // 8
    return torch.zeros(frames, slots, n // (frames * slots), dtype=torch.float64, device=device)


def gram_mse_ledger_supported(c):
    return bool(lib().maua_gram_mse_ledger_supported(int(c)))


def gram_fwd_mse_ledger(f, scale, center, out, mean_out, target, dmat, loss_scale, grad_scale, ledger, slot, workspace=None):
    c = f.shape[1] if f.dim() == 4 else f.shape[0]
    hw = f.numel() // c
    workspace = _ws(workspace, gram_workspace_bytes(c, hw), f.device)
    _check(lib().maua_gram_fwd_mse_ledger(_ptr(_f32(f, "f")), _ptr(out), _ptr(mean_out) if center else None, c, hw, float(scale),
                                          int(center), _ptr(_f32(target, "target")), _ptr(dmat), float(loss_scale),
                                          float(grad_scale), ledger.data_ptr(), int(slot), workspace.data_ptr(),
                                          workspace.numel() * workspace.element_size(), _stream()), "maua_gram_fwd_mse_ledger")
    return out


def gram_row_means(f, mean_out, workspace):
    c = f.shape[1] if f.dim() == 4 else f.shape[0]
    _check(lib().maua_gram_row_means(_ptr(_f32(f, "f")), _ptr(mean_out), c, f.numel() // c, workspace.data_ptr(),
                                     workspace.numel() * workspace.element_size(), _stream()), "maua_gram_row_means")


def gram_partial(f, center, mean_out, workspace):
    c = f.shape[1] if f.dim() == 4 else f.shape[0]
    hw = f.numel() // c
    _check(lib().maua_gram_partial(_ptr(_f32(f, "f")), _ptr(mean_out) if center else None, c, hw, int(center), workspace.data_ptr(),
                                   workspace.numel() * workspace.element_size(), _stream()), "maua_gram_partial")


class GramFinishBatch:

    def __init__(self, layers):
        n = len(layers)
        self.n = n
        self.keep = layers
        arr = lambda ct, vals: (ct * n)(*vals)
        self.args = (
            arr(ctypes.c_void_p, [l["workspace"].data_ptr() for l in layers]), arr(ctypes.c_void_p, [_ptr(l["gram"]) for l in layers]),
            arr(ctypes.c_void_p, [_ptr(_f32(l["target"], "target")) for l in layers]), arr(ctypes.c_void_p, [_ptr(l["dmat"]) for l in layers]),
            arr(ctypes.c_int, [int(l["c"]) for l in layers]), arr(ctypes.c_int64, [int(l["hw"]) for l in layers]),
            arr(ctypes.c_float, [float(l["scale"]) for l in layers]), arr(ctypes.c_float, [float(l["loss_scale"]) for l in layers]),
            arr(ctypes.c_float, [float(l["grad_scale"]) for l in layers]), arr(ctypes.c_void_p, [l["ledger"].data_ptr() for l in layers]),
            arr(ctypes.c_int, [int(l["slot"]) for l in layers]), arr(ctypes.c_int, [int(l.get("slabs") or 0) for l in layers]))

        self.partial_args = (
            arr(ctypes.c_void_p, [_ptr(_f32(l["f"], "f")) if l.get("f") is not None else None for l in layers]), self.args[4], self.args[5],
            self.args[0], arr(ctypes.c_size_t, [l["workspace"].numel() * l["workspace"].element_size() for l in layers]),
            arr(ctypes.c_void_p, [_ptr(l["mean"]) if l.get("mean") is not None else None for l in layers]))

    def run_partial(self):
        a = self.partial_args
        _check(lib().maua_gram_partial_batch(self.n, a[0], a[5], a[1], a[2], a[3], a[4], self.args[11], _stream()), "maua_gram_partial_batch")

    def run(self):
        a = self.args
        _check(lib().maua_gram_finish_mse_batch(self.n, a[0], a[1], a[2], a[3], a[4], a[5], a[6], a[7], a[8], a[9], a[10], a[11], _stream()),
               "maua_gram_finish_mse_batch")


def mse_fwd_bwd_ledger(x, target, grad, loss_scale, grad_scale, accumulate, ledger, slot, mask_grad_by_x=False):
    _check(lib().maua_mse_fwd_bwd_ledger(_ptr(_f32(x, "x")), _ptr(_f32(target, "target")), _ptr(grad), x.numel(), float(loss_scale),
                                         float(grad_scale), int(accumulate), int(mask_grad_by_x), ledger.data_ptr(), int(slot),
                                         _stream()), "maua_mse_fwd_bwd_ledger")


def tv_fwd_bwd_ledger(x, grad, strength, accumulate, ledger, slot):
    n, c, h, w = x.shape
    _check(lib().maua_tv_fwd_bwd_ledger(_ptr(_f32(x, "x")), _ptr(grad), n, c, h, w, float(strength), int(accumulate),
                                        ledger.data_ptr(), int(slot), _stream()), "maua_tv_fwd_bwd_ledger")


def loss_ledger_sum(ledger, losses, totals, losses_f64=None):
    frames, slots = ledger.shape[0], ledger.shape[1]
    if losses_f64 is not None:
        assert losses_f64.dtype == torch.float64 and losses_f64.numel() == frames * slots and losses_f64.is_contiguous()
        _check(lib().maua_loss_ledger_sum_f64(ledger.data_ptr(), frames, slots, _ptr(losses), _ptr(totals), losses_f64.data_ptr(),
                                              _stream()), "maua_loss_ledger_sum_f64")
        return
    _check(lib().maua_loss_ledger_sum(ledger.data_ptr(), frames, slots, _ptr(losses), _ptr(totals), _stream()),
           "maua_loss_ledger_sum")


def gram_bwd(d_sym, f, row_mean, gf, accumulate, workspace=None, relu_mask=None):
    c = d_sym.shape[0]
    hw = f.numel() // c
    workspace = _ws(workspace, 4 * c + 256, f.device)
    _check(lib().maua_gram_bwd(_ptr(_f32(d_sym, "d")), _ptr(f), _ptr(row_mean), _ptr(relu_mask), _ptr(gf), c, hw, int(accumulate),
                               workspace.data_ptr(), workspace.numel() * workspace.element_size(), _stream()),
           "maua_gram_bwd")
    return gf


def gram_guided_workspace_bytes(regions, c, hw):
    return lib().maua_gram_guided_workspace_bytes(int(regions), int(c), int(hw))


def _guides_2d(guides, hw):
    if guides.dim() < 2 or guides.numel() != guides.shape[0] * hw:
        raise HipError(f"guides of shape {tuple(guides.shape)} do not cover {hw} pixels per region")
    return guides.shape[0]


def gram_guided_mass(guides, out=None):
    r = guides.shape[0]
    hw = guides.numel() // max(r, 1)
    if out is None:
        out = torch.empty(r, dtype=torch.float64, device=guides.device)
    _check(lib().maua_gram_guided_mass(_ptr(_f32(guides, "guides")), _ptr(out), r, hw, _stream()), "maua_gram_guided_mass")
    return out


def gram_guided_fwd(f, guides, scale, center=False, mass=None, out=None, mean_out=None, workspace=None):
    c = f.shape[1] if f.dim() == 4 else f.shape[0]
    hw = f.numel() // c
    r = _guides_2d(guides, hw)
    if scale.numel() != r or (center and (mass is None or mass.numel() != r or mass.dtype != torch.float64)):
        raise HipError("gram_guided_fwd: one scale (float32) and, to centre, one mass (float64) per region")
    if out is None:
        out = torch.empty(r, c, c, device=f.device, dtype=torch.float32)
    if center and mean_out is None:
        mean_out = torch.empty(r, c, device=f.device, dtype=torch.float32)
    workspace = _ws(workspace, gram_guided_workspace_bytes(r, c, hw), f.device)
    _check(lib().maua_gram_guided_fwd(_ptr(_f32(f, "f")), _ptr(_f32(guides, "guides")), _ptr(_f32(scale, "scale")), _ptr(mass) if center else None,
                                      _ptr(out), _ptr(mean_out) if center else None, r, c, hw, int(center), workspace.data_ptr(),
                                      workspace.numel() * workspace.element_size(), _stream()), "maua_gram_guided_fwd")
    return out, (mean_out if center else None)


def gram_guided_bwd(d_sym, f, guides, coef, mean, gf, accumulate):
    r, c = d_sym.shape[0], d_sym.shape[1]
    hw = f.numel() // c
    if _guides_2d(guides, hw) != r or coef.numel() != r or gf.numel() != f.numel() or (mean is not None and mean.numel() != r * c):
        raise HipError("gram_guided_bwd: shapes of d_sym, guides, coef, mean and gf do not agree")
    _check(lib().maua_gram_guided_bwd(_ptr(_f32(d_sym, "d")), _ptr(_f32(f, "f")), _ptr(_f32(guides, "guides")), _ptr(_f32(coef, "coef")),
                                      _ptr(_f32(mean, "mean")), _ptr(_f32(gf, "gf")), r, c, hw, int(accumulate), _stream()), "maua_gram_guided_bwd")
    return gf


def gram_shift_supported(shifts, c, h, w):
    return bool(lib().maua_gram_shift_supported(int(shifts), int(c), int(h), int(w)))


def gram_shift_workspace_bytes(shifts, c, h, w):
    return lib().maua_gram_shift_workspace_bytes(int(shifts), int(c), int(h), int(w))


def _shift_args(shifts, factors):
    n = len(shifts)
    if n != len(factors):
        raise HipError(f"{n} shifts and {len(factors)} factors")
    return ((ctypes.c_int * n)(*[int(a) for a, _ in shifts]), (ctypes.c_int * n)(*[int(d) for _, d in shifts]),
            (ctypes.c_double * n)(*[float(v) for v in factors]))


def gram_shift_fwd(f, shifts, scales, mean=None, out=None, workspace=None):
    c, h, w = f.shape[-3], f.shape[-2], f.shape[-1]
    if f.numel() != c * h * w or (mean is not None and mean.numel() != c):
        raise HipError("gram_shift_fwd: f is one (C, H, W) map and mean holds C values")
    n = len(shifts)
    axes, deltas, fac = _shift_args(shifts, scales)
    if out is None:
        out = torch.empty(n, c, c, device=f.device, dtype=torch.float32)
    elif out.numel() != n * c * c:
# ... 555 lines not shown
        raise HipError(f"flow_warp_grid: flow of shape {tuple(flo.shape)}, expected (h, w, 2)")
    h, w = int(flo.shape[0]), int(flo.shape[1])
    oh, ow = int(size[0]), int(size[1])
    if oh <= 0 or ow <= 0:
        raise HipError(f"flow_warp_grid: output {oh}x{ow}")
    need = lib().maua_flow_warp_grid_workspace_bytes(h, w)
    if not need:
        raise HipError(f"flow_warp_grid: flow field {h}x{w}")
    grid = torch.empty(1, oh, ow, 2, device=flo.device, dtype=torch.float32)
    if workspace is None:
        workspace = torch.empty(need, dtype=torch.uint8, device=flo.device)
    _check(lib().maua_flow_warp_grid(_ptr(_f32(flo, "flo")), _ptr(grid), h, w, oh, ow, workspace.data_ptr(),
                                     workspace.numel() * workspace.element_size(), _stream()), "maua_flow_warp_grid")
    return grid


def grid_sample_border(x, grid, blend=None, blend_a=0.0):
    if x.dim() != 4 or grid.dim() != 4 or grid.shape[0] != x.shape[0] or grid.shape[3] != 2:
        raise HipError(f"grid_sample_border: x {tuple(x.shape)}, grid {tuple(grid.shape)}")
    n, c, h, w = (int(v) for v in x.shape)
    oh, ow = int(grid.shape[1]), int(grid.shape[2])
    out = torch.empty(n, c, oh, ow, device=x.device, dtype=torch.float32)
    init = None
    if blend is not None:
        if tuple(blend.shape) != tuple(x.shape) or (h, w) != (oh, ow):
            raise HipError(f"grid_sample_border: blend {tuple(blend.shape)} with x {tuple(x.shape)} sampled to {oh}x{ow}")
        init = torch.empty_like(out)
    _check(lib().maua_grid_sample_border(_ptr(_f32(x, "x")), _ptr(_f32(grid, "grid")), _ptr(out), n, c, h, w, oh, ow,
                                         _ptr(_f32(blend, "blend")), float(blend_a), _ptr(init), _stream()), "maua_grid_sample_border")
    return out if blend is None else (out, init)


def mask_u8_resize(mask, size):
    m = mask if mask.dim() == 3 else mask.unsqueeze(-1)
    if m.dim() != 3:
        raise HipError(f"mask_u8_resize: mask of shape {tuple(mask.shape)}")
    h, w, c = (int(v) for v in m.shape)
    oh, ow = int(size[0]), int(size[1])
    if oh <= 0 or ow <= 0:
        raise HipError(f"mask_u8_resize: output {oh}x{ow}")
    out = torch.empty(1, c, oh, ow, device=m.device, dtype=torch.float32)
    _check(lib().maua_mask_u8_resize(_u8(m, "mask"), _ptr(out), h, w, c, oh, ow, _stream()), "maua_mask_u8_resize")
    return out


def gauss_wrap(x, sigmas, roll=0, workspace=None, out=None):
    if not x.is_cuda:
        raise HipError("gauss_wrap: needs a ROCm device tensor (got a CPU tensor): there is no CPU path")
    if x.dim() != 4:
        raise HipError(f"gauss_wrap: clip of shape {tuple(x.shape)}, expected (T, C, H, W)")
    if len(sigmas) != 3:
        raise HipError(f"gauss_wrap: sigmas {sigmas!r}, expected (sigma_t, sigma_h, sigma_w)")
    t, c, h, w = (int(v) for v in x.shape)
    st, sh, sw = (float(v) for v in sigmas)
    L = lib()
    if not L.maua_gauss_wrap_supported(t, c, h, w, st, sh, sw):
        raise HipError(f"gauss_wrap: unsupported clip {tuple(x.shape)} with sigmas {(st, sh, sw)}")
    need = L.maua_gauss_wrap_workspace_bytes(t, c, h, w, st, sh, sw)
    if out is None:
        out = torch.empty_like(x, memory_format=torch.contiguous_format)
    elif tuple(out.shape) != tuple(x.shape):
        raise HipError(f"gauss_wrap: out {tuple(out.shape)} for a clip {tuple(x.shape)}")
    if workspace is None and need:
        workspace = torch.empty(need, dtype=torch.uint8, device=x.device)
    wp, wn = (workspace.data_ptr(), workspace.numel() * workspace.element_size()) if workspace is not None else (None, 0)
    _check(L.maua_gauss_wrap(_ptr(_f32(x, "x")), _ptr(_f32(out, "out")), t, c, h, w, st, sh, sw, int(roll) % t, wp, wn, _stream()), "maua_gauss_wrap")
    return out


class LbfgsState:

    def __init__(self, count, history, device):
        self.count, self.history = int(count), int(history)
        if not 0 < self.history <= 254:
            raise HipError(f"--lbfgs_num_correction {history}: the device-side recursion holds at most 254 pairs")
        nbytes = lib().maua_lbfgs_state_bytes(self.count, self.history)
        self.buf = torch.empty(nbytes, dtype=torch.uint8, device=device)
        self._status = torch.zeros(5, dtype=torch.float32, device=device)
        _check(lib().maua_lbfgs_init(self.buf.data_ptr(), nbytes, self.count, self.history, _stream()), "maua_lbfgs_init")

    def reset(self):
        _check(lib().maua_lbfgs_init(self.buf.data_ptr(), self.buf.numel(), self.count, self.history, _stream()), "maua_lbfgs_init")

    def iterate(self, x, grad, lr=1.0, tolerance_change=-1.0, tolerance_grad=-1.0, loss=None):
        _check(lib().maua_lbfgs_iterate(self.buf.data_ptr(), _ptr(x), _ptr(grad), _ptr(loss), self.count, self.history, float(lr),
                                        float(tolerance_change), float(tolerance_grad), _stream()), "maua_lbfgs_iterate")

    def status(self):
        _check(lib().maua_lbfgs_status(self.buf.data_ptr(), self.count, self.history, _ptr(self._status), _stream()),
               "maua_lbfgs_status")
        n_iter, hlen, stopped, gtd, t = self._status.tolist()
        return dict(n_iter=int(n_iter), history_len=int(hlen), stopped=bool(stopped), gtd=gtd, t=t)


FLOW_MAX_LEVELS = 8


def _flow_dims_ok(h, w):
    return 0 < h <= 1 << 16 and 0 < w <= 1 << 16 and h * w <= 1 << 28


def flow_levels(h, w, max_levels=5):
    if not _flow_dims_ok(h, w) or max_levels < 1:
        return 0
    n = 1
    while n < max_levels and (h + 1) // 2 >= 16 and (w + 1) // 2 >= 16:
        h, w, n = (h + 1) // 2, (w + 1) // 2, n + 1
    return n


def flow_tvl1_workspace_bytes(h, w, levels):
    if not _flow_dims_ok(h, w) or not 1 <= levels <= FLOW_MAX_LEVELS or levels > flow_levels(h, w, levels):
        return 0
    a = lambda b: (b + 255) & ~255
    total, lh, lw = 0, h, w
    for _ in range(levels):
        total += 2 * a(lh * lw * 4)
        lh, lw = (lh + 1) // 2, (lw + 1) // 2
    return total + 2 * a(6 * h * w * 4) + a(3 * h * w * 4) + a(2 * h * w * 4)


def _u8(t, name, shape=None):
    if not t.is_cuda or t.dtype != torch.uint8 or not t.is_contiguous():
        raise HipError(f"{name}: expected a contiguous uint8 device tensor")
    if shape is not None and tuple(t.shape) != tuple(shape):
        raise HipError(f"{name}: shape {tuple(t.shape)}, expected {tuple(shape)}")
    return t.data_ptr()


def flow_grey(rgb):
    h, w = rgb.shape[:2]
    out = torch.empty(h, w, dtype=torch.float32, device=rgb.device)
    _check(lib().maua_flow_grey_u8(_u8(rgb, "rgb", (h, w, 3)), out.data_ptr(), h, w, _stream()), "maua_flow_grey_u8")
    return out


def flow_pyr_down(img):
    h, w = img.shape
    out = torch.empty((h + 1) // 2, (w + 1) // 2, dtype=torch.float32, device=img.device)
    _check(lib().maua_flow_pyr_down(_ptr(_f32(img, "img")), out.data_ptr(), h, w, _stream()), "maua_flow_pyr_down")
    return out


def flow_warp_prep(i0, i1, u, fields=None):
    h, w = i0.shape
    if tuple(i1.shape) != (h, w) or tuple(u.shape) != (2, h, w):
        raise HipError("flow_warp_prep: shapes")
    if fields is None:
        fields = torch.empty(3, h, w, dtype=torch.float32, device=i0.device)
    _check(lib().maua_flow_warp_prep(_ptr(_f32(i0, "i0")), _ptr(_f32(i1, "i1")), _ptr(_f32(u, "u")), _ptr(fields), h, w, _stream()),
           "maua_flow_warp_prep")
    return fields


def flow_tvl1_step(fields, state, out=None, k=0):
    _, h, w = state.shape
    if tuple(state.shape) != (6, h, w) or tuple(fields.shape) != (3, h, w):
        raise HipError("flow_tvl1_step: shapes")
    if out is None:
        out = torch.empty_like(state)
    if k == 0:
        _check(lib().maua_flow_tvl1_step(_ptr(_f32(fields, "fields")), _ptr(_f32(state, "state")), _ptr(out), h, w, _stream()),
               "maua_flow_tvl1_step")
    else:
        _check(lib().maua_flow_tvl1_blocked(_ptr(_f32(fields, "fields")), _ptr(_f32(state, "state")), _ptr(out), h, w, int(k), _stream()),
               "maua_flow_tvl1_blocked")
    return out
# ... 112 lines not shown
```

maua-style_amd/optim.py:

```python
import json
import math
import os
import sys

import numpy as np
import torch as th
import tqdm

import config as config_mod
import engine as engine_mod
import hip
import loss as loss_mod
import plan
import models
from utils import limit_host_threads, wrapping_slice

PBAR = tqdm.tqdm(file=sys.stdout, smoothing=0.1, disable=not sys.stdout.isatty())


def _describe(text, args):
    if not args.verbose:
        PBAR.set_description(text)


# ... 190 lines not shown
            self.engine = getattr(net, "_maua_engine", None) or engine_mod.StyleEngine(net, losses)
            net._maua_engine = self.engine
        except engine_mod.UnsupportedNet:
            self.engine = None
        self.net, self.losses = net, losses
        self.x = _device_image(init, args).clone()
        self.kind = args.optimizer
        self.step_count = 0
        self.batch_hint = max(1, int(batch_hint))
        if self.engine is not None:
            self.engine.independent, self.engine.batch_hint = self.independent, self.batch_hint
        elif self.independent:
            raise engine_mod.UnsupportedNet("independent frame batches need the fused engine")
        self._bundle_key, bundle = None, None
        if self.engine is not None and self.kind == "lbfgs" and grad_hook is None and plan.on("graph_bundles"):
            self._bundle_key = ("lbfgs", tuple(self.x.shape), str(self.x.device), str(self.x.dtype), self.independent, self.batch_hint,
                                int(args.lbfgs_num_correction), float(args.lbfgs_tolerance_change), float(args.lbfgs_tolerance_grad))
            try:
                self.engine._prepare(self.x)
            except engine_mod.UnsupportedNet:
                if self.independent:
                    raise
                self.engine, self._bundle_key = None, None
        if self._bundle_key is not None:
            bundle = self.engine.iter_graphs.get(self._bundle_key)
            if bundle is not None and (bundle["epoch"] != self.engine.alloc_epoch or bundle["graph_key"] != self.engine._graph_key()):
                bundle = None
                del self.engine.iter_graphs[self._bundle_key]
            owner = bundle.get("owner") if bundle is not None else None
            if owner is not None and owner() is not None and owner() is not self:
                bundle = None
            elif bundle is not None:
                import weakref
                bundle["owner"] = weakref.ref(self)
        if bundle is not None:
            bundle["x"].copy_(self.x)
            self.x = bundle["x"]
        self.frames = [self.x[b] for b in range(self.x.shape[0])] if self.independent else [self.x]
        if self.kind == "lbfgs":
            if bundle is not None:
                self.states = bundle["states"]
                for st in self.states:
                    st.reset()
            else:
                self.states = [hip.LbfgsState(f.numel(), int(args.lbfgs_num_correction), self.x.device) for f in self.frames]
            self.state = self.states[0]
        elif self.kind == "adam":
            self.m, self.v = th.zeros_like(self.x), th.zeros_like(self.x)
        else:
            raise ValueError(f"unknown optimizer {self.kind}")
        hg = getattr(args, "hip_graph", None)
        if hg is None:
            enough = planned_iters is None or planned_iters >= (GRAPH_MIN_ITERS_REPEATED if repeated and self._bundle_key else GRAPH_MIN_ITERS)
            hg = plan.on("hip_graph") and (enough or bundle is not None)
        self.use_graph = bool(hg)
        self._graph = bundle["graph"] if (bundle is not None and self.use_graph) else None
        self._keep_bundle = bool(repeated) and self._bundle_key is not None
        self.owns_x = bundle is None and not self._keep_bundle

    def feval(self):
        if self.engine is not None:
            self.engine.independent, self.engine.batch_hint = self.independent, self.batch_hint
            try:
                return self.engine.feval(self.x, capture=self.use_graph and self.kind != "lbfgs" and self.engine.timer is None)
            except engine_mod.UnsupportedNet:
                self.engine = None
        return self._feval_modules()

    def _feval_modules(self):
        x = self.x.detach().requires_grad_(True)
        self.net(x)
        total = 0
        slots = th.zeros(max(len(self.losses), 1), device=x.device)
        for idx, mod in enumerate(self.losses):
            if isinstance(mod.loss, int) and mod.loss == 0:
                continue
            slots[idx] = mod.loss.detach()
            total = total + mod.loss
        total.backward()
        for mod in self.losses:
            mod.loss = 0
        return slots, total.detach().reshape(1), x.grad.contiguous()

    def _lbfgs_move(self, grad, total):
        a = self.args
        eng = self.engine if self.independent else None
        if eng is not None:
            eng.fork()
        for b, (st, xf) in enumerate(zip(self.states, self.frames)):
            gb = grad[b] if self.independent else grad
            lb = None
            if th.is_tensor(total) and total.is_cuda:
                lb = total[b:b + 1] if self.independent else total
            if eng is not None:
                ctx, _ = eng.frame_stream(b)
                with ctx:
                    st.iterate(xf, gb, 1.0, float(a.lbfgs_tolerance_change), float(a.lbfgs_tolerance_grad), lb)
            else:
                st.iterate(xf, gb, 1.0, float(a.lbfgs_tolerance_change), float(a.lbfgs_tolerance_grad), lb)
        if eng is not None:
            eng.join()

    def stopped(self):
        return self.kind == "lbfgs" and all(st.status()["stopped"] for st in self.states)

    def _step_lbfgs_graph(self):
        if self._graph is not None:
            self._graph.replay()
            self.step_count += 1
            return self.engine.slots, self.engine.total
        slots, total, grad = self.engine.feval(self.x)
        if self.grad_hook is not None:
            self.grad_hook(grad)
        self._lbfgs_move(grad, total)
        self.step_count += 1
        th.cuda.synchronize()
        graph = th.cuda.CUDAGraph()
        with th.cuda.graph(graph):
            self.engine._run(self.x)
            if self.grad_hook is not None:
                self.grad_hook(self.engine.gbuf[0])
            self._lbfgs_move(self.engine.gbuf[0], self.engine.total)
        self._graph = graph
        if self._keep_bundle:
            import weakref
            self.engine.iter_graphs[self._bundle_key] = {"graph": graph, "x": self.x, "states": self.states, "epoch": self.engine.alloc_epoch,
                                                         "graph_key": self.engine._graph_key(), "owner": weakref.ref(self)}
        return slots, total

    def step(self):
        if self.use_graph and self.kind == "lbfgs" and self.engine is not None and self.engine.timer is None:
            try:
                return self._step_lbfgs_graph()
            except engine_mod.UnsupportedNet:
                self.engine = None
        slots, total, grad = self.feval()
        if self.grad_hook is not None:
            self.grad_hook(grad)
        self.step_count += 1
        a = self.args
        if self.kind == "lbfgs":
            self._lbfgs_move(grad, total)
        else:
            hip.adam_step(self.x, grad, self.m, self.v, self.step_count, float(a.learning_rate))
        return slots, total


def _run_iterations(opt, num_iters, args, save_offset=0, save_total=None):
    if args.optimizer == "lbfgs":
        _describe("Running optimization with L-BFGS", args)
        steps = lbfgs_moves(num_iters)
    else:
        _describe("Running optimization with ADAM", args)
        steps = num_iters + 1
    for i in range(1, steps + 1):
        if args.save_iter > 0 and (i % args.save_iter == 0 or i == num_iters):
            import load
            last = save_offset + i == (save_total if save_total is not None else num_iters)
            load.save_tensor_to_file(opt.x.detach().cpu(), args, None if last else save_offset + i, opt.x.size(3))
        slots, total = opt.step()
        if not args.verbose and not (args.optimizer == "adam" and i == 1):
            PBAR.update(1)
        if args.print_iter > 0 and i % args.print_iter == 0 and args.verbose:
            print(f"Iteration {i} / {args.num_iters}, Loss: {float(total.sum())}")
        if args.optimizer == "lbfgs" and i % 25 == 0 and opt.stopped():
            break


def video_windows(init, styles, window):
    num_windows = math.ceil(init.shape[0] / window)
    seqs = [init] + list(styles)
    framestep = np.array([seq.shape[0] - window / 2 for seq in seqs]) / num_windows
    return [[math.ceil(framestep[k] * n) for n in range(num_windows + 1)] if seq.shape[0] != 1 else [0] * (num_windows + 1)
            for k, seq in enumerate(seqs)]


def _optimize_video(content, styles, init, num_iters, args, net=None, losses=None, keep_on_device=False):
    limit_host_threads()
    on_device = bool(keep_on_device) and init.is_cuda
    window = int(args.gram_frame_window)
    windows = video_windows(init, styles, window)
    if net is None or losses is None:
        set_model_args(args, max(*init.shape))
        net, losses = models.load_model(args)
    if not args.verbose:
        PBAR.reset()
        PBAR.total = len(windows[0]) * num_iters
        PBAR.refresh()
    set_content_targets(net, content, args)
    if args.avg_frame_window == -1:
        set_style_video_targets(net, styles, args)
        for mod in losses:
            mod.mode = "loss"

    output = init.clone()
    for w, window_start in enumerate(windows[0]):
        front_overlap = windows[0][w - 1] + window - window_start
        end_overlap = (window_start + window) % output.shape[0] if window_start + window >= output.shape[0] else 0
        index = wrapping_slice(output, window_start, window, return_indices=True)
        if args.avg_frame_window != -1:
            current_styles = [wrapping_slice(style, windows[k + 1][w], args.avg_frame_window) for k, style in enumerate(styles)]
            set_style_video_targets(net, current_styles, args)
            for mod in losses:
                mod.mode = "loss"
        if w == 0 and args.normalize_weights:
# ... 116 lines not shown
```

maua-style_amd/plan.py:

```python
import os
import sys

FIELDS = {
    "conv_x6": ("1", "host", "3x3 stride-1 layers on the reduced-width matrix cores with fp32-accurate operand splits: 1 both passes, fwd / bwd one pass, 0 fp32 MFMA"),
    "conv_x3": ("1", "host", "1: fp16x3 arithmetic (22 significand bits, conv_x3*.hip); 0: bf16x6 everywhere (the strictly 24-bit route bench.py reports beside the headline)"),
    "conv_x3w": ("1", "host", "layers whose consumed channel count is a multiple of 16 run conv_x3w.hip instead of conv_x3.hip"),
    "conv_x3q": ("256", "host", "smallest consumed channel count from which a 3x3 layer runs conv_x3q.hip (0: never)"),
    "conv_x3p": ("64", "host", "smallest consumed channel count from which a 3x3 layer may run the persistent conv_x3p.hip (0: never); conv_x3p_preferred decides per launch"),
    "conv_x3p_max": ("100000", "host", "largest consumed channel count for conv_x3p.hip"),
    "x3p_gram_min_mb": ("700", "host", "the Gram backward rides in conv_x3p's launch from this many MB of maps per launch (below: conv_x3w's fused form)"),
    "conv_image": ("1", "host", "the 3-channel image layer's forward pass on conv_img.hip"),
    "split_min_produced": ("16", "host", "a 3x3 stride-1 pass runs the split-precision kernels (64-channel tiles) when it PRODUCES at least this many channels, else the fp32-MFMA / direct kernels (VGG-19 / NIN: only the 64 -> 3 image gradient is below; the pruned VGG-16 has widths of 22 and 24)"),
    "x3w_min_pixels": ("4096", "host", "planes smaller than this run conv_x3.hip's 4-row tiles"),
    "few_mfma": ("1", "host", "backward-data of the image layer (64 -> 3 channels) on the matrix cores (conv_few_mfma.hip) instead of conv3x3_few_out's vector-ALU kernel"),
    "strided_fwd_3x3": ("1", "host", "forward pass of a strided, unpadded layer (NIN's stem) as space to depth + a stride-1 3x3 convolution over sites (conv_x3w)"),
    "strided_bwd_3x3": ("1", "host", "backward-data of a strided, unpadded layer (NIN's 11x11 / 4 stem) as a stride-1 3x3 convolution over the output sites + depth to space"),
    "pool_codes": ("1", "host", "2x2 / 2 max pools keep one decision byte per window for the backward pass"),
    "loss_ledger": ("1", "host", "loss partial sums go to a ledger summed once per evaluation"),
    "gram_batch": ("1", "host", "one finishing launch for the Gram / loss chains of all style layers"),
    "gram_partial_batch": ("1", "host", "one partial-product launch for the Gram-form layers"),
    "fuse_pool": ("1", "host", "conv + ReLU + pool in one launch where the pool is the activation's only consumer"),
    "fuse_pool_split": ("1", "host", "... also where the small grid splits the channel loop (the adding pass pools)"),
    "fuse_unpool": ("1", "host", "backward-data staged straight from the pooled map's gradient and the decision bytes"),
    "fuse_gram_max_c": ("256", "host", "style layers of at most this many channels have their Gram backward ride in the next convolution's backward launch (0: never)"),
    "image_gram": ("1", "host", "the image layer's launch leaves the Gram slabs of relu1_1"),
    "finish_in_launch": ("0", "host", "1: the engine arms its split-K workspace - small splits are added up by the last workgroup to arrive at a tile, no finishing launch (bit-identical; measured neutral at 512 x 512: the last arriver's serial chain costs what the launch cost, profiles/probes_r06.md section 1)"),
    "dmat_pack_batch": ("1", "host", "one launch packs the D matrices of all fused style layers"),
    "style_stream": ("auto", "host", "Gram / loss chains of a single image on a side stream: 0, 1, or auto (from 1536 x 1536 pixels)"),
    "side_streams": ("4", "host", "side streams for the per-frame kernels of independent frames (0: none)"),
    "hip_graph": ("1", "host", "replay iterations from captured hipGraphs"),
    "graph_bundles": ("1", "host", "L-BFGS iterations captured as whole bundles (evaluation + update)"),
    "frame_batch": ("0", "host", "vid_img: frames per batch (0: planned from memory; 1: the reference's frame-by-frame loop)"),
    "frame_cache_mb": ("4096", "host", "vid_img: host cache for decoded frames"),
    "temporal_device": ("0", "host", "vid_img over a flow cache: 1 keeps frames, warp grid, reliability mask and blend on the device (csrc/warp.hip; frames chain through the 8-bit image the PNG holds), 0 the reference's host loop"),
    "clip_device": ("0", "host", "img_vid: 1 keeps the clip on the device between and inside scales (initial filter and temporal blend in csrc/gauss_wrap.hip, windows gathered on the device, frames leave as 8-bit images), 0 the reference's host loop"),
    "guided_engine": ("0", "host", "img_img with guides (spatial control): 1 runs the guided style layers inside the fused engine and its captured graph (per-region Gram, loss and D matrices in one finishing launch, csrc/gram_guided.hip; B = 1, needs loss_ledger), 0 the module path"),
    "debug_poison": ("0", "host", "tests: every engine buffer starts as NaN"),
    "conv_few_out": ("1", "lib", "3x3 passes that produce <= 4 channels run conv3x3_few_out (0: the general MFMA kernel)"),
    "few_out_ks4_below": ("1024", "lib", "conv3x3_few_out: launches of fewer workgroups than this split the channel loop four ways"),
    "x3w_ks": ("0", "lib", "conv_x3w: force this K split (0: cost model)"),
    "x3w_stagger": ("7", "lib", "conv_x3w: start delay of odd-slot workgroups, units of 512 cycles"),
    "finish_in_launch_max_ks": ("4", "lib", "split channel loops of at most this many slabs are finished inside the producing launch when the workspace is armed (conv_x3q, conv_x3w)"),
    "x3q_ks": ("0", "lib", "conv_x3q: force this K split (0: cost model)"),
    "x3q_min_fill": ("0.85", "lib", "conv_x3q_preferred: smallest grid fill x plane cover"),
    "x3q_min_chunks": ("4", "lib", "conv_x3q_preferred: smallest number of 32-channel chunks per workgroup"),
    "x3p_ks": ("0", "lib", "conv_x3p: force this K split (0: cost model)"),
    "gram_mask_reuse": ("1", "lib", "conv_x3w with the fused Gram backward, whole chunk list: the masked epilogue takes the bits F > 0 from the Gram phase's operand registers (0: it loads F again)"),
    "cot_inner": ("0", "lib", "conv_x3w / conv_x3q workgroup order: 1 = the channel tiles of a pixel tile start side by side on one XCD (shared patch in its L2), 0 = blockIdx.y is the channel tile"),
    "x3p_order": ("1", "lib", "conv_x3p's work list: 0 channel tile outermost (an XCD's band = part of one channel tile's plane), 1 pixel tile outermost (the channel tiles of a pixel tile side by side on an XCD's CUs: the plane leaves memory once)"),
    "x3p_groups": ("256", "lib", "conv_x3p: workgroups per launch (a multiple of 8)"),
    "x3p_min_fill": ("0.8", "lib", "conv_x3p_preferred: smallest list fill x plane cover"),
    "x3p_min_items": ("512", "lib", "conv_x3p_preferred: smallest number of work items (and a quarter of the smallest items x chunks)"),
    "x6_persist": ("0", "lib", "conv_x6: several tiles per workgroup (experiment)"),
    "gram_x3": ("1", "lib", "Gram partial products in fp16x3 (0: fp32 MFMA)"),
    "gram_bwd_x3": ("1", "lib", "Gram backward in fp16x3 (0: fp32 MFMA)"),
    "gram_t128": ("1", "lib", "128 x 128 two-role Gram blocks: 0 never, 1 whole 64-pixel stages, 2 ragged maps too"),
    "gram_t128_min_hw": ("1024", "lib", "128 x 128 Gram blocks from this many pixels"),
    "p1_order": ("1", "lib", "conv1x1_x3: (pixel tile, channel tile) items in XCD bands, channel tiles adjacent (0: dispatch order)"),
    "lbfgs_vec": ("1", "lib", "lbfgs: 16-byte loads in the history sweeps"),
    "lbfgs_tri": ("1", "lib", "lbfgs: the triangular form of the coefficient kernel"),
}

ENV_VARS = {
    "MAUA_HIP_LIB": None,
    "MAUA_PLAN": None,
    "MAUA_CONV_X3": "conv_x3",
    "MAUA_CONV_X6": "conv_x6",
    "MAUA_HIP_GRAPH": "hip_graph",
    "MAUA_DEBUG_POISON": "debug_poison",
    "MAUA_DIST_BACKEND": None,
    "MAUA_DIST_TIMEOUT_S": None,
    "MAUA_DIST_JOB_TIMEOUT_S": None,
    "MAUA_HOST_THREADS": None,
}
_FIELD_VAR = {field: var for var, field in ENV_VARS.items() if field is not None}
_TOOL_VARS = {"MAUA_FUZZ_ASSUME_NO_GPU"}

OVERRIDES = {}


_plan_cache = (None, {})


def _planned():
    global _plan_cache
    text = os.environ.get("MAUA_PLAN")
    if _plan_cache[0] != text or text is None:
        _plan_cache = (text, _parse_plan(text))
    return _plan_cache[1]


def _parse_plan(text):
    out = {}
    for part in (text or "").replace(";", ",").split(","):
        part = part.strip()
        if not part:
            continue
        if "=" not in part:
            raise ValueError(f"MAUA_PLAN: expected field=value, got {part!r}")
        k, v = part.split("=", 1)
        k = k.strip().lower()
        if k.startswith("maua_"):
            k = k[5:]
        if k not in FIELDS:
            raise ValueError(f"MAUA_PLAN: unknown field {k!r} (plan.FIELDS lists them)")
        out[k] = v.strip()
    return out


def get(name):
    default = FIELDS[name][0]
    if name in OVERRIDES:
        return str(OVERRIDES[name])
    planned = _planned()
    if name in planned:
        return planned[name]
    var = _FIELD_VAR.get(name)
    if var is not None and var in os.environ:
        return os.environ[var]
    return default


def get_int(name):
    return int(float(get(name)))


def get_float(name):
    return float(get(name))


def on(name):
    return get(name) != "0"


def in_effect():
    return {k: get(k) for k in FIELDS if get(k) != FIELDS[k][0]}


def ignored_variables(environ=None):
    environ = os.environ if environ is None else environ
    return sorted(k for k in environ if k.startswith("MAUA_") and k not in ENV_VARS and k not in _TOOL_VARS)


# ... 25 lines not shown
```

Before: 201.7.

## Co-launch the loss ledger sum with the L-BFGS pair update and drop slot fill

Adds a generic co-launch template that runs two independent kernel bodies in one grid. The loss-ledger summing pass now shares a launch with the L-BFGS pair-update kernel inside the captured graph. A 'fresh' mode makes the summing pass write every loss slot, so the engine can skip the fill of the slot buffer before each evaluation. This removes a launch and a fill per iteration. In exchange, the pair kernel's blocks run at the ledger body's 1024-thread block size and launch bounds, which may change its occupancy.

Result: no change. 202.1 (median of 6 runs) (+0.2%).

```diff
diff --git a/include/maua_hip.h b/include/maua_hip.h
--- a/include/maua_hip.h
+++ b/include/maua_hip.h
@@ -242,6 +242,8 @@
 int maua_loss_ledger_sum(double* ledger, int frames, int slots, float* losses, float* totals, maua_stream_t stream);
 int maua_loss_ledger_sum_f64(double* ledger, int frames, int slots, float* losses, float* totals, double* losses_f64,
                              maua_stream_t stream);
+int maua_loss_ledger_sum_fresh(double* ledger, int frames, int slots, float* losses, float* totals, double* losses_f64,
+                               maua_stream_t stream);
 
 int maua_fill(float* x, int64_t count, float value, maua_stream_t stream);
 size_t maua_conv_few_mfma_bank_bytes(void);
@@ -295,6 +297,9 @@
 int maua_lbfgs_init(void* state, size_t state_bytes, int64_t count, int history, maua_stream_t stream);
 int maua_lbfgs_iterate(void* state, float* x, const float* grad, const float* loss, int64_t count, int history, float lr,
                        float tolerance_change, float tolerance_grad, maua_stream_t stream);
+int maua_lbfgs_iterate_ledger(void* state, float* x, const float* grad, const float* loss, int64_t count, int history, float lr,
+                              float tolerance_change, float tolerance_grad, double* ledger, int frames, int slots, float* losses,
+                              float* totals, double* losses_f64, int fresh, maua_stream_t stream);
 int maua_lbfgs_status(const void* state, int64_t count, int history, float* out5, maua_stream_t stream);
 
 int maua_flow_levels(int h, int w, int max_levels);
diff --git a/maua-style_amd/csrc/co_launch.hpp b/maua-style_amd/csrc/co_launch.hpp
--- /dev/null
+++ b/maua-style_amd/csrc/co_launch.hpp
@@ -0,0 +1,38 @@
+#pragma once
+#include "common.hpp"
+
+namespace maua {
+
+template <class A, class B>
+struct CoLaunch {
+    static constexpr int THREADS = A::THREADS > B::THREADS ? A::THREADS : B::THREADS;
+    static constexpr int PER_A = THREADS / A::THREADS, PER_B = THREADS / B::THREADS;
+    static constexpr int WAVES = A::WAVES > B::WAVES ? A::WAVES : B::WAVES;
+    static_assert(A::THREADS % 64 == 0 && B::THREADS % 64 == 0 && THREADS % A::THREADS == 0 && THREADS % B::THREADS == 0,
+                  "co-launch: block sizes must be multiples of 64 and divide the larger one");
+    static_assert((!A::BARRIERS || PER_A == 1) && (!B::BARRIERS || PER_B == 1), "co-launch: a body with barriers must own the whole block");
+    static int blocks_a(int na) { return (na + PER_A - 1) / PER_A; }
+    static int blocks_b(int nb) { return (nb + PER_B - 1) / PER_B; }
+};
+
+template <class A, class B>
+__global__ void __launch_bounds__((CoLaunch<A, B>::THREADS), (CoLaunch<A, B>::WAVES)) co_launch_kernel(typename A::Args a, int na, typename B::Args b, int nb) {
+    using C = CoLaunch<A, B>;
+    const int split = (na + C::PER_A - 1) / C::PER_A;
+    if ((int)blockIdx.x < split) {
+        const int v = (int)blockIdx.x * C::PER_A + (int)threadIdx.x / A::THREADS;
+        if (v < na) A::run(a, v, na, (int)threadIdx.x % A::THREADS);
+    } else {
+        const int v = ((int)blockIdx.x - split) * C::PER_B + (int)threadIdx.x / B::THREADS;
+        if (v < nb) B::run(b, v, nb, (int)threadIdx.x % B::THREADS);
+    }
+}
+
+template <class A, class B>
+inline void co_launch(const typename A::Args& a, int na, const typename B::Args& b, int nb, hipStream_t stream) {
+    using C = CoLaunch<A, B>;
+    const int grid = C::blocks_a(na) + C::blocks_b(nb);
+    if (grid > 0) hipLaunchKernelGGL((co_launch_kernel<A, B>), dim3(grid), dim3(C::THREADS), 0, stream, a, na, b, nb);
+}
+
+}
diff --git a/maua-style_amd/csrc/conv_api.hip b/maua-style_amd/csrc/conv_api.hip
--- a/maua-style_amd/csrc/conv_api.hip
+++ b/maua-style_amd/csrc/conv_api.hip
@@ -16,7 +16,7 @@
 namespace maua {
 static const char* const g_tuning_names[] = {"conv_few_out", "few_out_ks4_below", "x3w_ks", "x3w_stagger", "x3q_ks", "x3q_min_fill", "x3q_min_chunks",
                                              "x3p_ks", "x3p_groups", "x3p_min_fill", "x3p_min_items", "x6_persist", "gram_x3", "gram_bwd_x3",
-                                             "gram_t128", "gram_t128_min_hw", "p1_order", "lbfgs_vec", "lbfgs_tri", "finish_in_launch_max_ks", "x3p_order", "cot_inner", "gram_mask_reuse"};
+                                             "gram_t128", "gram_t128_min_hw", "p1_order", "lbfgs_vec", "lbfgs_tri", "finish_in_launch_max_ks", "x3p_order", "cot_inner", "gram_mask_reuse", "co_launch"};
 constexpr int kTunings = sizeof(g_tuning_names) / sizeof(g_tuning_names[0]);
 static double g_tuning_values[kTunings];
 static bool g_tuning_set[kTunings];
diff --git a/maua-style_amd/csrc/lbfgs.hip b/maua-style_amd/csrc/lbfgs.hip
--- a/maua-style_amd/csrc/lbfgs.hip
+++ b/maua-style_amd/csrc/lbfgs.hip
@@ -1,7 +1,9 @@
 #include <stdint.h>
 #include <stdlib.h>
 
+#include "co_launch.hpp"
 #include "common.hpp"
+#include "loss_ledger.hpp"
 
 #ifndef LB_NT
 #define LB_NT 1
@@ -109,19 +111,34 @@
     }
 }
 
-__global__ void __launch_bounds__(256)
-lbfgs_pair_kernel(const LbfgsHeader* __restrict__ hdr, const float* __restrict__ g, float* __restrict__ g_prev,
-                  const float* __restrict__ d, float* __restrict__ S, float* __restrict__ Y, int64_t n) {
-    const bool first = hdr->n_iter == 0;
-    const float t = hdr->t;
-    float* sc = S + (int64_t)hdr->cand * n;
-    float* yc = Y + (int64_t)hdr->cand * n;
-    for (int64_t e = (int64_t)blockIdx.x * blockDim.x + threadIdx.x; e < n; e += (int64_t)gridDim.x * blockDim.x) {
-        const float gv = g[e];
-        sc[e] = first ? 0.f : d[e] * t;
-        yc[e] = first ? 0.f : gv - g_prev[e];
-        g_prev[e] = gv;
-    }
+struct LbfgsPairBody {
+    struct Args {
+        const LbfgsHeader* hdr;
+        const float* g;
+        float* g_prev;
+        const float* d;
+        float* S;
+        float* Y;
+        int64_t n;
+    };
+    static constexpr int THREADS = 256;
+    static constexpr bool BARRIERS = false;
+    static constexpr int WAVES = 8;
+    static __device__ __forceinline__ void run(const Args& a, int block, int nblocks, int tid) {
+        const bool first = a.hdr->n_iter == 0;
+        const float t = a.hdr->t;
+        float* sc = a.S + (int64_t)a.hdr->cand * a.n;
+        float* yc = a.Y + (int64_t)a.hdr->cand * a.n;
+        for (int64_t e = (int64_t)block * THREADS + tid; e < a.n; e += (int64_t)nblocks * THREADS) {
+            const float gv = a.g[e];
+            sc[e] = first ? 0.f : a.d[e] * t;
+            yc[e] = first ? 0.f : gv - a.g_prev[e];
+            a.g_prev[e] = gv;
+        }
+    }
+};
+__global__ void __launch_bounds__(LbfgsPairBody::THREADS) lbfgs_pair_kernel(LbfgsPairBody::Args a) {
+    LbfgsPairBody::run(a, blockIdx.x, gridDim.x, threadIdx.x);
 }
 
 template <bool VEC>
@@ -735,26 +752,8 @@
 
 using namespace maua;
 
-extern "C" {
-
-size_t maua_lbfgs_state_bytes(int64_t count, int history) {
-    if (count <= 0 || history <= 0 || history > 254 || count >= (1ll << 36)) return 0;
-    return lbfgs_layout(count, history).total;
-}
-
-int maua_lbfgs_init(void* state, size_t state_bytes, int64_t count, int history, maua_stream_t stream) {
-    MAUA_REQUIRE(state && count > 0 && count < (1ll << 36) && history > 0 && history <= 254, MAUA_E_INVAL, "lbfgs_init: bad args");
-    MAUA_REQUIRE(2 * (history + 1) + 1 <= 512, MAUA_E_UNSUPPORTED, "lbfgs_init: history %d too large (at most 254)", history);
-    const LbfgsLayout L = lbfgs_layout(count, history);
-    MAUA_REQUIRE(state_bytes >= L.total, MAUA_E_WORKSPACE, "lbfgs_init: state %zu < %zu bytes", state_bytes, L.total);
-    char* b = (char*)state;
-    hipLaunchKernelGGL(lbfgs_init_kernel, dim3(64), dim3(256), 0, (hipStream_t)stream, (LbfgsHeader*)b,
-                       (double*)(b + L.off_M), L.nb_ids, (float*)(b + L.off_coef));
-    return check_launch("lbfgs_init_kernel");
-}
-
-int maua_lbfgs_iterate(void* state, float* x, const float* grad, const float* loss, int64_t count, int history, float lr,
-                       float tolerance_change, float tolerance_grad, maua_stream_t stream) {
+static int lbfgs_iterate_impl(void* state, float* x, const float* grad, const float* loss, int64_t count, int history, float lr,
+                              float tolerance_change, float tolerance_grad, const LedgerSumBody::Args* led, int frames, maua_stream_t stream) {
     MAUA_REQUIRE(state && x && grad && count > 0 && count < (1ll << 36) && history > 0 && history <= 254, MAUA_E_INVAL, "lbfgs_iterate: bad args");
     const LbfgsLayout L = lbfgs_layout(count, history);
     char* b = (char*)state;
@@ -772,8 +771,19 @@
     MAUA_REQUIRE(lds1 <= 64 * 1024 && L.nb_ids <= 512, MAUA_E_UNSUPPORTED, "lbfgs_iterate: history %d too large (at most 254)", history);
     int pg = (int)((count + 1023) / 1024);
     if (pg > 2048) pg = 2048;
-    hipLaunchKernelGGL(lbfgs_pair_kernel, dim3(pg), dim3(256), 0, s, hdr, grad, g_prev, d, S, Y, count);
-    int rc = check_launch("lbfgs_pair_kernel");
+    const LbfgsPairBody::Args pair{hdr, grad, g_prev, d, S, Y, count};
+    int rc;
+    if (led && tuning("co_launch", 1) != 0) {
+        co_launch<LedgerSumBody, LbfgsPairBody>(*led, frames, pair, pg, s);
+        rc = check_launch("co_launch_kernel<LedgerSumBody, LbfgsPairBody>");
+    } else {
+        if (led && frames > 0) {
+            rc = loss_ledger_sum_launch(*led, frames, s);
+            if (rc) return rc;
+        }
+        hipLaunchKernelGGL(lbfgs_pair_kernel, dim3(pg), dim3(256), 0, s, pair);
+        rc = check_launch("lbfgs_pair_kernel");
+    }
     if (rc) return rc;
     int groups = (1024 + L.nwg - 1) / L.nwg;
     if (groups > L.m1) groups = L.m1;
@@ -817,6 +827,38 @@
     return check_launch("lbfgs_combine_kernel");
 }
 
+extern "C" {
+
+size_t maua_lbfgs_state_bytes(int64_t count, int history) {
+    if (count <= 0 || history <= 0 || history > 254 || count >= (1ll << 36)) return 0;
+    return lbfgs_layout(count, history).total;
+}
+
+int maua_lbfgs_init(void* state, size_t state_bytes, int64_t count, int history, maua_stream_t stream) {
+    MAUA_REQUIRE(state && count > 0 && count < (1ll << 36) && history > 0 && history <= 254, MAUA_E_INVAL, "lbfgs_init: bad args");
+    MAUA_REQUIRE(2 * (history + 1) + 1 <= 512, MAUA_E_UNSUPPORTED, "lbfgs_init: history %d too large (at most 254)", history);
+    const LbfgsLayout L = lbfgs_layout(count, history);
+    MAUA_REQUIRE(state_bytes >= L.total, MAUA_E_WORKSPACE, "lbfgs_init: state %zu < %zu bytes", state_bytes, L.total);
+    char* b = (char*)state;
+    hipLaunchKernelGGL(lbfgs_init_kernel, dim3(64), dim3(256), 0, (hipStream_t)stream, (LbfgsHeader*)b,
+                       (double*)(b + L.off_M), L.nb_ids, (float*)(b + L.off_coef));
+    return check_launch("lbfgs_init_kernel");
+}
+
+int maua_lbfgs_iterate(void* state, float* x, const float* grad, const float* loss, int64_t count, int history, float lr,
+                       float tolerance_change, float tolerance_grad, maua_stream_t stream) {
+    return lbfgs_iterate_impl(state, x, grad, loss, count, history, lr, tolerance_change, tolerance_grad, nullptr, 0, stream);
+}
+
+int maua_lbfgs_iterate_ledger(void* state, float* x, const float* grad, const float* loss, int64_t count, int history, float lr,
+                              float tolerance_change, float tolerance_grad, double* ledger, int frames, int slots, float* losses,
+                              float* totals, double* losses_f64, int fresh, maua_stream_t stream) {
+    MAUA_REQUIRE(frames == 0 || (ledger && losses && totals && frames > 0 && frames <= (1 << 16) && slots > 0 && slots <= (1 << 12)),
+                 MAUA_E_INVAL, "lbfgs_iterate_ledger: bad args");
+    const LedgerSumBody::Args led{ledger, slots, losses, totals, losses_f64, fresh ? 1 : 0};
+    return lbfgs_iterate_impl(state, x, grad, loss, count, history, lr, tolerance_change, tolerance_grad, &led, frames, stream);
+}
+
 #ifdef LB_STAMP
 int maua_lbfgs_read_stamps(unsigned long long* host16) {
     return (int)hipMemcpyFromSymbol(host16, HIP_SYMBOL(g_lb_stamps), sizeof(unsigned long long) * 16);
diff --git a/maua-style_amd/csrc/loss_ledger.hpp b/maua-style_amd/csrc/loss_ledger.hpp
--- /dev/null
+++ b/maua-style_amd/csrc/loss_ledger.hpp
@@ -0,0 +1,68 @@
+#pragma once
+#include "common.hpp"
+
+namespace maua {
+
+constexpr int LEDGER_GROUPS = 4;
+struct LedgerSumBody {
+    struct Args {
+        double* ledger;
+        int slots;
+        float* losses;
+        float* total;
+        double* exact;
+        int fresh;
+    };
+    static constexpr int THREADS = 256 * LEDGER_GROUPS;
+    static constexpr bool BARRIERS = true;
+    static constexpr int WAVES = 4;
+    static __device__ __forceinline__ void run(const Args& a, int frame, int , int tid) {
+        __shared__ double scratch[LEDGER_GROUPS][4];
+        __shared__ float kept[1 << 12];
+        const int slots = a.slots;
+        double* led = a.ledger + (int64_t)frame * slots * LEDGER_STRIDE;
+        float* out = a.losses + (int64_t)frame * slots;
+        const int grp = tid >> 8, t = tid & 255, lane = t & 63, wave = t >> 6;
+        constexpr int PER = LEDGER_MAX / 256;
+        for (int s0 = 0; s0 < slots; s0 += LEDGER_GROUPS) {
+            const int s = s0 + grp;
+            const bool have = s < slots;
+            const double* rec = led + (int64_t)(have ? s : 0) * LEDGER_STRIDE;
+            double part[PER];
+#pragma unroll
+            for (int i = 0; i < PER; ++i) part[i] = rec[2 + t + 256 * i];
+            const int n = have ? min((int)rec[0], LEDGER_MAX) : 0;
+            double v = 0.0;
+#pragma unroll
+            for (int i = 0; i < PER; ++i) v += t + 256 * i < n ? part[i] : 0.0;
+            v = wave_sum(v);
+            if (lane == 0) scratch[grp][wave] = v;
+            __syncthreads();
+            if (t == 0 && have) {
+                if (n > 0) {
+                    double r = 0.0;
+                    for (int i = 0; i < 4; ++i) r += scratch[grp][i];
+                    const double scl = rec[1];
+                    kept[s] = (float)(r * scl);
+                    out[s] = kept[s];
+                    if (a.exact) a.exact[(int64_t)frame * slots + s] = r * scl;
+                    led[(int64_t)s * LEDGER_STRIDE] = 0.0;
+                } else if (a.fresh) {
+                    kept[s] = 0.f;
+                    out[s] = 0.f;
+                } else {
+                    kept[s] = out[s];
+                }
+            }
+            __syncthreads();
+        }
+        if (tid == 0) {
+            float tot = 0.f;
+            for (int s = 0; s < slots; ++s) tot += kept[s];
+            a.total[frame] = tot;
+        }
+    }
+};
+int loss_ledger_sum_launch(const LedgerSumBody::Args& a, int frames, hipStream_t stream);
+
+}
diff --git a/maua-style_amd/csrc/pointwise.hip b/maua-style_amd/csrc/pointwise.hip
--- a/maua-style_amd/csrc/pointwise.hip
+++ b/maua-style_amd/csrc/pointwise.hip
@@ -1,6 +1,7 @@
 #include <stdarg.h>
 
 #include "common.hpp"
+#include "loss_ledger.hpp"
 
 namespace maua {
 
@@ -21,50 +22,12 @@
     if (threadIdx.x == 0) out[0] = (float)(v * (double)scale);
 }
 
-constexpr int LEDGER_GROUPS = 4;
-__global__ void __launch_bounds__(256 * LEDGER_GROUPS)
-loss_ledger_sum_kernel(double* __restrict__ ledger, int slots, float* __restrict__ losses, float* __restrict__ total,
-                       double* __restrict__ exact) {
-    __shared__ double scratch[LEDGER_GROUPS][4];
-    __shared__ float kept[1 << 12];
-    double* led = ledger + (int64_t)blockIdx.x * slots * LEDGER_STRIDE;
-    float* out = losses + (int64_t)blockIdx.x * slots;
-    const int grp = threadIdx.x >> 8, t = threadIdx.x & 255, lane = t & 63, wave = t >> 6;
-    constexpr int PER = LEDGER_MAX / 256;
-    for (int s0 = 0; s0 < slots; s0 += LEDGER_GROUPS) {
-        const int s = s0 + grp;
-        const bool have = s < slots;
-        const double* rec = led + (int64_t)(have ? s : 0) * LEDGER_STRIDE;
-        double part[PER];
-#pragma unroll
-        for (int i = 0; i < PER; ++i) part[i] = rec[2 + t + 256 * i];
-        const int n = have ? min((int)rec[0], LEDGER_MAX) : 0;
-        double v = 0.0;
-#pragma unroll
-        for (int i = 0; i < PER; ++i) v += t + 256 * i < n ? part[i] : 0.0;
-        v = wave_sum(v);
-        if (lane == 0) scratch[grp][wave] = v;
-        __syncthreads();
-        if (t == 0 && have) {
-            if (n > 0) {
-                double r = 0.0;
-                for (int i = 0; i < 4; ++i) r += scratch[grp][i];
-                const double scl = rec[1];
-                kept[s] = (float)(r * scl);
-                out[s] = kept[s];
-                if (exact) exact[(int64_t)blockIdx.x * slots + s] = r * scl;
-                led[(int64_t)s * LEDGER_STRIDE] = 0.0;
-            } else {
-                kept[s] = out[s];
-            }
-        }
-        __syncthreads();
-    }
-    if (threadIdx.x == 0) {
-        float tot = 0.f;
-        for (int s = 0; s < slots; ++s) tot += kept[s];
-        total[blockIdx.x] = tot;
-    }
+__global__ void __launch_bounds__(LedgerSumBody::THREADS) loss_ledger_sum_kernel(LedgerSumBody::Args a) {
+    LedgerSumBody::run(a, blockIdx.x, gridDim.x, threadIdx.x);
+}
+int loss_ledger_sum_launch(const LedgerSumBody::Args& a, int frames, hipStream_t stream) {
+    hipLaunchKernelGGL(loss_ledger_sum_kernel, dim3(frames), dim3(LedgerSumBody::THREADS), 0, stream, a);
+    return check_launch("loss_ledger_sum_kernel");
 }
 
 __global__ void pack_filters_kernel(const float* __restrict__ w, float* __restrict__ wf, float* __restrict__ wb, int cout,
@@ -647,21 +610,26 @@
     return check_launch("tv_kernel");
 }
 
+static int ledger_sum_launch(const char* who, double* ledger, int frames, int slots, float* losses, float* totals, double* losses_f64,
+                             int fresh, maua_stream_t stream) {
+    MAUA_REQUIRE(ledger && losses && totals && frames > 0 && frames <= (1 << 16) && slots > 0 && slots <= (1 << 12), MAUA_E_INVAL,
+                 "%s: bad args", who);
+    return loss_ledger_sum_launch(LedgerSumBody::Args{ledger, slots, losses, totals, losses_f64, fresh}, frames, (hipStream_t)stream);
+}
+
 int maua_loss_ledger_sum(double* ledger, int frames, int slots, float* losses, float* totals, maua_stream_t stream) {
-    MAUA_REQUIRE(ledger && losses && totals && frames > 0 && frames <= (1 << 16) && slots > 0 && slots <= (1 << 12), MAUA_E_INVAL,
-                 "loss_ledger_sum: bad args");
-    hipLaunchKernelGGL(loss_ledger_sum_kernel, dim3(frames), dim3(256 * LEDGER_GROUPS), 0, (hipStream_t)stream, ledger, slots, losses, totals,
-                       (double*)nullptr);
-    return check_launch("loss_ledger_sum_kernel");
+    return ledger_sum_launch("loss_ledger_sum", ledger, frames, slots, losses, totals, nullptr, 0, stream);
 }
 
 int maua_loss_ledger_sum_f64(double* ledger, int frames, int slots, float* losses, float* totals, double* losses_f64,
                              maua_stream_t stream) {
-    MAUA_REQUIRE(ledger && losses && totals && losses_f64 && frames > 0 && frames <= (1 << 16) && slots > 0 && slots <= (1 << 12),
-                 MAUA_E_INVAL, "loss_ledger_sum_f64: bad args");
-    hipLaunchKernelGGL(loss_ledger_sum_kernel, dim3(frames), dim3(256 * LEDGER_GROUPS), 0, (hipStream_t)stream, ledger, slots, losses, totals,
-                       losses_f64);
-    return check_launch("loss_ledger_sum_kernel");
+    MAUA_REQUIRE(losses_f64, MAUA_E_INVAL, "loss_ledger_sum_f64: bad args");
+    return ledger_sum_launch("loss_ledger_sum_f64", ledger, frames, slots, losses, totals, losses_f64, 0, stream);
+}
+
+int maua_loss_ledger_sum_fresh(double* ledger, int frames, int slots, float* losses, float* totals, double* losses_f64,
+                               maua_stream_t stream) {
+    return ledger_sum_launch("loss_ledger_sum_fresh", ledger, frames, slots, losses, totals, losses_f64, 1, stream);
 }
 
 int maua_depth_to_space(const float* in, float* out, int n, int c_out, int r, int qh, int qw, int h, int w, int accumulate, maua_stream_t stream) {
diff --git a/maua-style_amd/engine.py b/maua-style_amd/engine.py
--- a/maua-style_amd/engine.py
+++ b/maua-style_amd/engine.py
@@ -587,12 +587,30 @@
     def _x6_ok(self, s, produced_channels):
         return self.use_x6 and s.k == 3 and s.stride == 1 and s.pad <= 2 and produced_channels >= plan.get_int("split_min_produced")
 
-    def _run(self, x):
+    def _ledger_owns_slots(self):
+        if self.ledger is None or not plan.on("co_launch"):
+            return False
+        for s in self.steps:
+            if s.kind == "content" and s.mod.weights is not None:
+                return False
+            if s.kind == "style" and id(s) not in self.guided and not hip.gram_mse_ledger_supported(self.act[s.src].shape[1]):
+                return False
+        return True
+
+    def deferred_ledger(self):
+        return self.ledger, self.slots_all, self.total, self.slots_f64, self._ledger_owns_slots()
+
+    def can_defer_ledger(self):
+        return self.ledger is not None and self.ledger.shape[0] == 1 and not self.term_steps
+
+    def _run(self, x, defer_ledger=False):
         hip.set_split_batch_hint(self.batch_hint)
         self._arm()
         a, g = self.act, self.gbuf
         a[0] = x
-        hip.fill_(self.slots_all, 0.0)
+        fresh = self._ledger_owns_slots()
+        if not fresh:
+            hip.fill_(self.slots_all, 0.0)
         forked = False
         batch = []
         emitted = set()
@@ -977,7 +995,10 @@
         if cur != 0:
             hip.fill_(g[0], 0.0)
         if self.ledger is not None:
-            hip.loss_ledger_sum(self.ledger, self.slots_all, self.total, self.slots_f64)
+            if defer_ledger:
+                assert self.can_defer_ledger()
+                return
+            hip.loss_ledger_sum(self.ledger, self.slots_all, self.total, self.slots_f64, fresh=fresh)
             for s in self.steps:
                 td = self.term_steps.get(id(s))
                 if td is not None and self._active(s, a[s.src].shape):
diff --git a/maua-style_amd/hip.py b/maua-style_amd/hip.py
--- a/maua-style_amd/hip.py
+++ b/maua-style_amd/hip.py
@@ -164,9 +164,11 @@
     "maua_gram_row_means": (c_i, [c_p, c_p, c_i, c_i64, c_p, c_sz, c_p]),
     "maua_loss_ledger_sum": (c_i, [c_p, c_i, c_i, c_p, c_p, c_p]),
     "maua_loss_ledger_sum_f64": (c_i, [c_p, c_i, c_i, c_p, c_p, c_p, c_p]),
+    "maua_loss_ledger_sum_fresh": (c_i, [c_p, c_i, c_i, c_p, c_p, c_p, c_p]),
     "maua_lbfgs_state_bytes": (c_sz, [c_i64, c_i]),
     "maua_lbfgs_init": (c_i, [c_p, c_sz, c_i64, c_i, c_p]),
     "maua_lbfgs_iterate": (c_i, [c_p, c_p, c_p, c_p, c_i64, c_i, c_f, c_f, c_f, c_p]),
+    "maua_lbfgs_iterate_ledger": (c_i, [c_p, c_p, c_p, c_p, c_i64, c_i, c_f, c_f, c_f, c_p, c_i, c_i, c_p, c_p, c_p, c_i, c_p]),
     "maua_lbfgs_status": (c_i, [c_p, c_i64, c_i, c_p, c_p]),
     "maua_flow_levels": (c_i, [c_i, c_i, c_i]),
     "maua_flow_grey_u8": (c_i, [c_p, c_p, c_i, c_i, c_p]),
@@ -797,15 +799,21 @@
                                         ledger.data_ptr(), int(slot), _stream()), "maua_tv_fwd_bwd_ledger")
 
 
-def loss_ledger_sum(ledger, losses, totals, losses_f64=None):
+def _ledger_args(ledger, losses, totals, losses_f64):
     frames, slots = ledger.shape[0], ledger.shape[1]
     if losses_f64 is not None:
         assert losses_f64.dtype == torch.float64 and losses_f64.numel() == frames * slots and losses_f64.is_contiguous()
-        _check(lib().maua_loss_ledger_sum_f64(ledger.data_ptr(), frames, slots, _ptr(losses), _ptr(totals), losses_f64.data_ptr(),
-                                              _stream()), "maua_loss_ledger_sum_f64")
-        return
-    _check(lib().maua_loss_ledger_sum(ledger.data_ptr(), frames, slots, _ptr(losses), _ptr(totals), _stream()),
-           "maua_loss_ledger_sum")
+    return ledger.data_ptr(), frames, slots, _ptr(losses), _ptr(totals)
+
+
+def loss_ledger_sum(ledger, losses, totals, losses_f64=None, fresh=False):
+    args = _ledger_args(ledger, losses, totals, losses_f64)
+    if fresh:
+        _check(lib().maua_loss_ledger_sum_fresh(*args, _ptr(losses_f64), _stream()), "maua_loss_ledger_sum_fresh")
+    elif losses_f64 is not None:
+        _check(lib().maua_loss_ledger_sum_f64(*args, losses_f64.data_ptr(), _stream()), "maua_loss_ledger_sum_f64")
+    else:
+        _check(lib().maua_loss_ledger_sum(*args, _stream()), "maua_loss_ledger_sum")
 
 
 def gram_bwd(d_sym, f, row_mean, gf, accumulate, workspace=None, relu_mask=None):
@@ -1527,7 +1535,13 @@
     def reset(self):
         _check(lib().maua_lbfgs_init(self.buf.data_ptr(), self.buf.numel(), self.count, self.history, _stream()), "maua_lbfgs_init")
 
-    def iterate(self, x, grad, lr=1.0, tolerance_change=-1.0, tolerance_grad=-1.0, loss=None):
+    def iterate(self, x, grad, lr=1.0, tolerance_change=-1.0, tolerance_grad=-1.0, loss=None, ledger=None):
+        if ledger is not None:
+            led, losses, totals, losses_f64, fresh = ledger
+            _check(lib().maua_lbfgs_iterate_ledger(self.buf.data_ptr(), _ptr(x), _ptr(grad), _ptr(loss), self.count, self.history, float(lr),
+                                                   float(tolerance_change), float(tolerance_grad), *_ledger_args(led, losses, totals, losses_f64),
+                                                   _ptr(losses_f64), int(bool(fresh)), _stream()), "maua_lbfgs_iterate_ledger")
+            return
         _check(lib().maua_lbfgs_iterate(self.buf.data_ptr(), _ptr(x), _ptr(grad), _ptr(loss), self.count, self.history, float(lr),
                                         float(tolerance_change), float(tolerance_grad), _stream()), "maua_lbfgs_iterate")
 
diff --git a/maua-style_amd/optim.py b/maua-style_amd/optim.py
--- a/maua-style_amd/optim.py
+++ b/maua-style_amd/optim.py
@@ -296,7 +296,7 @@
             mod.loss = 0
         return slots, total.detach().reshape(1), x.grad.contiguous()
 
-    def _lbfgs_move(self, grad, total):
+    def _lbfgs_move(self, grad, total, ledger=None):
         a = self.args
         eng = self.engine if self.independent else None
         if eng is not None:
@@ -311,7 +311,7 @@
                 with ctx:
                     st.iterate(xf, gb, 1.0, float(a.lbfgs_tolerance_change), float(a.lbfgs_tolerance_grad), lb)
             else:
-                st.iterate(xf, gb, 1.0, float(a.lbfgs_tolerance_change), float(a.lbfgs_tolerance_grad), lb)
+                st.iterate(xf, gb, 1.0, float(a.lbfgs_tolerance_change), float(a.lbfgs_tolerance_grad), lb, ledger=ledger)
         if eng is not None:
             eng.join()
 
@@ -330,11 +330,12 @@
         self.step_count += 1
         th.cuda.synchronize()
         graph = th.cuda.CUDAGraph()
+        defer = plan.on("co_launch") and not self.independent and len(self.states) == 1 and self.engine.can_defer_ledger()
         with th.cuda.graph(graph):
-            self.engine._run(self.x)
+            self.engine._run(self.x, defer_ledger=defer)
             if self.grad_hook is not None:
                 self.grad_hook(self.engine.gbuf[0])
-            self._lbfgs_move(self.engine.gbuf[0], self.engine.total)
+            self._lbfgs_move(self.engine.gbuf[0], self.engine.total, ledger=self.engine.deferred_ledger() if defer else None)
         self._graph = graph
         if self._keep_bundle:
             import weakref
diff --git a/maua-style_amd/plan.py b/maua-style_amd/plan.py
--- a/maua-style_amd/plan.py
+++ b/maua-style_amd/plan.py
@@ -59,6 +59,7 @@
     "p1_order": ("1", "lib", "conv1x1_x3: (pixel tile, channel tile) items in XCD bands, channel tiles adjacent (0: dispatch order)"),
     "lbfgs_vec": ("1", "lib", "lbfgs: 16-byte loads in the history sweeps"),
     "lbfgs_tri": ("1", "lib", "lbfgs: the triangular form of the coefficient kernel"),
+    "co_launch": ("1", "lib", "independent neighbouring small kernels share a launch (the loss ledger's summing pass rides with the L-BFGS pair update), and that pass writes every loss slot, so the engine drops the fill in front of an evaluation (0: separate launches and the fill; same bits)"),
 }
 
 ENV_VARS = {
```
